# FlyCole/Dream2Real

Hardware: AMD Instinct MI355X
Metric: candidate renders scored/sec (640x360) (higher is better)
Workload: dtype bf16 + fp16 NeRF MLP operands (fp32 accumulate; the library's default: the reference's tiny-cuda-nn operand type, same MFMA rate; --opt mlp_f16=0 = bf16 operands)

## Files before the change

dream2real_amd/_lib.py:

```python
from __future__ import annotations

import ctypes as C
import os

import numpy as np

_HERE = os.path.dirname(os.path.abspath(__file__))
LIB_PATH = os.path.join(_HERE, "libd2r.so")
ABI_VERSION = 10

_int, _u32, _i64, _u64, _size, _f32, _f64, _str, _ptr = (C.c_int, C.c_uint32, C.c_int64, C.c_uint64, C.c_size_t, C.c_float, C.c_double,
                                                          C.c_char_p, C.c_void_p)
PROTOTYPES = {
    "d2r_abi_version": (_int, ()),
    "d2r_ctx_create": (_int, (_int, _ptr)),
    "d2r_ctx_destroy": (None, (_ptr,)),
    "d2r_ctx_set_stream": (_int, (_ptr, _ptr)),
    "d2r_ctx_synchronize": (_int, (_ptr,)),
    "d2r_last_error": (_str, (_ptr,)),
    "d2r_nerf_create": (_int, (_ptr, _ptr, _ptr)),
    "d2r_nerf_destroy": (None, (_ptr,)),
    "d2r_nerf_load_ingp": (_int, (_ptr, _ptr, _size, _ptr, _ptr, _ptr, _u32)),
    "d2r_ingp_inspect": (_int, (_ptr, _size, _ptr, _size, _ptr)),
    "d2r_ingp_validate": (_int, (_ptr, _size, _ptr)),
# ... 69 lines not shown
    "d2r_png_read_grey": (_int, (_str, _u32, _u32, _u32, _ptr)),
    "d2r_scene_bound_masks": (_int, (_ptr, _ptr, _u32, _u32, _u32, _ptr, _ptr, _ptr, _u32, _ptr, _ptr)),
    "d2r_masks_prune": (_int, (_ptr, _int, _ptr, _ptr, _ptr, _u32, _u32, _u32, _ptr, _ptr, _ptr, _u32, _ptr)),
    "d2r_masks_components": (_int, (_ptr, _ptr, _ptr, _u32, _u32, _ptr, _ptr, _ptr)),
    "d2r_masks_lut": (_int, (_ptr, _ptr, _ptr, _u32, _u32, _u32, _ptr, _ptr, _ptr)),
    "d2r_masks_census": (_int, (_ptr, _ptr, _u32, _u32, _u32, _ptr)),
    "d2r_masks_get_timing": (_int, (_ptr, _ptr)),
    "d2r_thumbs_plan": (_int, (_ptr, _ptr, _ptr, _ptr, _u32, _u32, _u32, _u32, _ptr, _ptr, _ptr, _ptr)),
    "d2r_thumbs_fill": (_int, (_ptr, _ptr, _ptr, _u64)),
    "d2r_thumbs_blur_bits": (_int, (_ptr, _ptr, _u32, _u32, _u32, _ptr)),
    "d2r_thumbs_get_timing": (_int, (_ptr, _ptr)),
    "d2r_proposals_labels": (_int, (_ptr, _ptr, _ptr, _u32, _u32, _u32, _ptr, _ptr, _ptr)),
    "d2r_proposals_get_timing": (_int, (_ptr, _ptr)),
    "d2r_labeltrack_grid": (_int, (_ptr, _ptr, _ptr, _ptr)),
    "d2r_labeltrack_scan": (_int, (_ptr, _ptr, _ptr, _u32, _u32, _u32, _ptr, _ptr, _ptr, _ptr, _ptr, _ptr, _ptr, _ptr, _ptr)),
    "d2r_labeltrack_get_timing": (_int, (_ptr, _ptr)),
    "d2r_geoprop_masks": (_int, (_ptr, _ptr, _ptr, _ptr, _u32, _u32, _ptr, _ptr, _ptr, _ptr, _ptr, _ptr, _ptr)),
    "d2r_geoprop_get_timing": (_int, (_ptr, _ptr)),
}
EXPORTS = list(PROTOTYPES)


class D2RError(RuntimeError):
    pass


class NerfDesc(C.Structure):
    _fields_ = [("n_levels", C.c_uint32), ("n_features", C.c_uint32), ("level_scale", C.c_void_p),
                ("level_res", C.c_void_p), ("level_size", C.c_void_p), ("level_offset", C.c_void_p),
                ("n_entries", C.c_uint32), ("grid_fp16", C.c_void_p), ("dw1_fp16", C.c_void_p),
                ("dw2_fp16", C.c_void_p), ("cw1_fp16", C.c_void_p), ("cw2_fp16", C.c_void_p),
                ("cw3_fp16", C.c_void_p), ("occupancy_bits", C.c_void_p), ("aabb_scale", C.c_uint32),
                ("render_aabb", C.c_float * 6)]


class ViewC(C.Structure):
    _fields_ = [("width", C.c_uint32), ("height", C.c_uint32), ("focal", C.c_float * 2),
                ("center", C.c_float * 2), ("scale", C.c_float), ("offset", C.c_float * 3),
                ("background", C.c_float * 4), ("min_transmittance", C.c_float),
                ("near_distance", C.c_float), ("lens_mode", C.c_uint32), ("lens_params", C.c_float * 4)]


class ClipDesc(C.Structure):
    _fields_ = [("image_size", C.c_uint32), ("patch_size", C.c_uint32), ("hidden_size", C.c_uint32),
                ("num_layers", C.c_uint32), ("num_heads", C.c_uint32), ("mlp_size", C.c_uint32),
                ("proj_dim", C.c_uint32)]


class TextDesc(C.Structure):
    _fields_ = [("vocab_size", C.c_uint32), ("context_length", C.c_uint32), ("hidden_size", C.c_uint32),
                ("num_layers", C.c_uint32), ("num_heads", C.c_uint32), ("mlp_size", C.c_uint32),
                ("proj_dim", C.c_uint32)]


class PhysParams(C.Structure):
    _fields_ = [("sample_res", C.c_uint32 * 6), ("init_pose", C.c_float * 16), ("table_z", C.c_float),
                ("unsup_thresh", C.c_float), ("gravity", C.c_float * 3), ("perturb", C.c_float),
                ("stability_check", C.c_int32), ("disallow_regrasp", C.c_int32), ("margin", C.c_float)]


class IngpView(C.Structure):
    _fields_ = [("fx", C.c_double), ("fy", C.c_double), ("cx", C.c_double), ("cy", C.c_double), ("w", C.c_uint32), ("h", C.c_uint32),
                ("lens_mode", C.c_uint32), ("lens_params", C.c_float * 4)]


class IngpInfo(C.Structure):
    _fields_ = [("n_levels", C.c_uint32), ("n_features", C.c_uint32), ("aabb_scale", C.c_uint32),
                ("has_background", C.c_int32), ("dataset_scale", C.c_double), ("dataset_offset", C.c_double * 3),
                ("background_color", C.c_float * 4), ("n_views", C.c_uint32), ("n_views_written", C.c_uint32),
                ("n_unknown_keys", C.c_uint32), ("render_with_lens_distortion", C.c_int32)]


class PcdView(C.Structure):
    _fields_ = [("width", C.c_uint32), ("height", C.c_uint32), ("fx", C.c_float), ("fy", C.c_float), ("cx", C.c_float),
                ("cy", C.c_float), ("point_size", C.c_float), ("near", C.c_float)]


class FrameSink(C.Structure):
    _fields_ = [("png_dir", C.c_char_p), ("png_first_index", C.c_uint32), ("png_threads", C.c_int32), ("png_level", C.c_int32)]


class RenderStats(C.Structure):
    _fields_ = [("rays_total", C.c_uint64), ("rays_alive", C.c_uint64), ("samples", C.c_uint64),
                ("wave_iters", C.c_uint64), ("l0_tokens", C.c_uint64), ("l0_touched", C.c_uint64)]


class Timing(C.Structure):
    _fields_ = [("march_ms", C.c_double), ("march_launches", C.c_uint64), ("raygen_ms", C.c_double),
                ("raygen_launches", C.c_uint64), ("prep_ms", C.c_double), ("prep_launches", C.c_uint64),
                ("clip_ms", C.c_double), ("clip_launches", C.c_uint64), ("sort_ms", C.c_double), ("sort_launches", C.c_uint64),
                ("vit_qkv_ms", C.c_double), ("vit_qkv_launches", C.c_uint64), ("vit_attn_ms", C.c_double), ("vit_attn_launches", C.c_uint64),
                ("vit_out_ms", C.c_double), ("vit_out_launches", C.c_uint64), ("vit_fc1_ms", C.c_double), ("vit_fc1_launches", C.c_uint64),
                ("vit_fc2_ms", C.c_double), ("vit_fc2_launches", C.c_uint64)]


COMM_ID_BYTES = 128

_lib = None


def load() -> C.CDLL:
    global _lib
    if _lib is not None:
        return _lib
    if not os.path.exists(LIB_PATH):
        raise D2RError(f"{LIB_PATH} is missing: build it with __graft_entry__.build() "
                       "(make -C dream2real_amd/csrc); there is no CPU fallback")
    try:
        import torch
    except ImportError:
        pass
    lib = C.CDLL(LIB_PATH)
    for name, (restype, argtypes) in PROTOTYPES.items():
        fn = getattr(lib, name)
        fn.restype, fn.argtypes = restype, argtypes
    if lib.d2r_abi_version() != ABI_VERSION:
        raise D2RError("libd2r.so ABI version mismatch")
    _lib = lib
    return lib


def ingp_inspect(data: bytes) -> str:
    lib = load()
    need = C.c_size_t(0)
    check(lib.d2r_ingp_inspect(data, len(data), None, 0, C.byref(need)))
    buf = C.create_string_buffer(need.value)
    check(lib.d2r_ingp_inspect(data, len(data), buf, need.value, None))
    return buf.value.decode("utf-8", "replace")


def png_write(rgb, path: str, level: int = -1):
    a = np.ascontiguousarray(rgb, np.uint8)
    assert a.ndim == 3 and a.shape[2] == 3
    check(load().d2r_png_write(ptr(a), a.shape[1], a.shape[0], os.fsencode(path), level))


def png_write_batch(frames, out_dir: str, first_index: int = 0, threads: int = 0, level: int = -1):
    a = np.ascontiguousarray(frames, np.uint8)
    assert a.ndim == 4 and a.shape[3] == 3
    check(load().d2r_png_write_batch(ptr(a), a.shape[0], a.shape[2], a.shape[1], os.fsencode(out_dir), first_index, threads, level))


def png_write_batch_bg(frames, background, out_dir: str, first_index: int = 0, threads: int = 0):
    a = np.ascontiguousarray(frames, np.uint8)
    b = np.ascontiguousarray(background, np.uint8)
    assert a.ndim == 4 and a.shape[3] == 3 and b.shape == a.shape[1:]
    check(load().d2r_png_write_batch_bg(ptr(a), a.shape[0], a.shape[2], a.shape[1], ptr(b), os.fsencode(out_dir), first_index, threads))


def png_write_channels(pixels, path: str, level: int = -1):
    a = np.ascontiguousarray(pixels, np.uint8)
    if a.ndim == 2:
        a = a[:, :, None]
    if a.ndim != 3 or a.shape[2] not in (1, 3, 4):
        raise ValueError(f"expected [h,w], [h,w,3] or [h,w,4], got shape {a.shape}")
    check(load().d2r_png_write_channels(ptr(a), a.shape[1], a.shape[0], a.shape[2], os.fsencode(path), level))


def png_info(path: str):
    v = [C.c_uint32(0) for _ in range(4)]
    check(load().d2r_png_info(os.fsencode(path), *[C.byref(x) for x in v]))
    return tuple(int(x.value) for x in v)


def png_read_rgb(path: str, size=None) -> np.ndarray:
    w, h = size or png_info(path)[:2]
    out = np.empty((h, w, 3), np.uint8)
# ... 286 lines not shown
```

dream2real_amd/csrc/api.hip:

```cpp
#include <math.h>
#include <string.h>

#include <algorithm>
#include <chrono>

#include "d2r_internal.h"
#include "pngio.h"

struct d2r_clip;
int d2r_launch_preprocess(d2r_ctx *, d2r_clip *, const uint8_t *frames_dev, uint32_t n, uint32_t w, uint32_t h,
                          int rot90, uint16_t *patches_dev, float *pixel_values_dev, const void *rects_dev = nullptr,
                          const uint16_t *bg_patches_dev = nullptr, bool touched_only = false);
bool d2r_clip_l0_supported(const d2r_ctx *, const d2r_clip *);
int d2r_clip_forward(d2r_ctx *, const d2r_clip *, const uint16_t *patches_dev, uint32_t n, const float *text_dev,
                     uint32_t C, float logit_scale, float *logits_dev, float *embeds_dev, const ClipL0Reuse *reuse = nullptr);
int d2r_clip_layer0_background(d2r_ctx *, const d2r_clip *, const uint16_t *bg_patches_dev, ClipL0Reuse *out);
int d2r_launch_patchify(d2r_ctx *, const d2r_clip *, const float *pv_dev, uint32_t n, uint16_t *patches_dev);
size_t d2r_clip_patch_bytes(const d2r_clip *, uint32_t n);
int d2r_launch_eval_points(d2r_ctx *, const d2r_nerf *, const float *xyz, const float *dirs, uint32_t n, float *out);
uint32_t d2r_clip_image_size(const d2r_clip *);
uint32_t d2r_clip_proj_dim(const d2r_clip *);
uint32_t d2r_clip_max_images(const d2r_clip *);
uint32_t d2r_clip_tokens(const d2r_clip *);

uint32_t d2r_pass_size(const d2r_ctx *ctx, const d2r_clip *clip, size_t px)
{
    uint64_t per = (uint64_t)std::max<int64_t>(1, ctx->chunk);
    if (clip) per = std::min<uint64_t>(per, d2r_clip_max_images(clip));
    if (px) per = std::min<uint64_t>(per, std::max<uint64_t>(1, 0xffffffffull / px));
    return (uint32_t)per;
}

static thread_local std::string g_err;

int d2r_fail(d2r_ctx *ctx, int code, const std::string &msg)
{
    if (ctx) ctx->err = msg;
    g_err = msg;
    return code;
}

hipStream_t d2r_stream(const d2r_ctx *ctx) { return ctx->stream; }

int d2r_reserve(d2r_ctx *ctx, d2r_ctx::Buf &b, size_t bytes)
{
    if (bytes <= b.cap) return D2R_OK;
    if (b.p) {
        D2R_HIP(ctx, hipStreamSynchronize(ctx->stream));
        (void)hipFree(b.p);
        b.p = nullptr;
        b.cap = 0;
    }
    size_t want = bytes + bytes / 8 + 256;
    if (hipMalloc(&b.p, want) != hipSuccess) {
        b.p = nullptr;
        return d2r_fail(ctx, D2R_ERR_MEMORY, "hipMalloc(" + std::to_string(want) + ") failed");
    }
    b.cap = want - 64;
    D2R_HIP(ctx, hipMemsetAsync(b.p, 0, want, ctx->stream));
    return D2R_OK;
}

uint32_t d2r_frame_pass_size(uint32_t per, size_t px)
{
    const uint64_t fit = std::max<uint64_t>(64, (1ull << 30) / (px * 3));
    uint64_t p = std::min<uint64_t>(per, fit);
    if (p >= 256) p -= p % 256;
    return (uint32_t)std::max<uint64_t>(1, p);
}

int d2r_upload_text(d2r_ctx *ctx, const d2r_clip *clip, const float *text, uint32_t C)
{
    if (!text || C == 0 || C > 1024) return d2r_fail(ctx, D2R_ERR_INVALID, "bad text embeddings");
    size_t bytes = (size_t)C * d2r_clip_proj_dim(clip) * 4;
    int rc = d2r_reserve(ctx, ctx->text, bytes);
    if (rc) return rc;
    const uint32_t slot = ctx->text_turn++ & 1u;
    if (ctx->text_ev[slot]) D2R_HIP(ctx, hipEventSynchronize(ctx->text_ev[slot]));
    else D2R_HIP(ctx, hipEventCreateWithFlags(&ctx->text_ev[slot], hipEventDisableTiming));
    if (ctx->text_host_cap[slot] < bytes) {
        if (ctx->text_host[slot]) (void)hipHostFree(ctx->text_host[slot]);
        ctx->text_host[slot] = nullptr;
        ctx->text_host_cap[slot] = 0;
        if (hipHostMalloc(&ctx->text_host[slot], bytes + 4096, hipHostMallocDefault) != hipSuccess)
            return d2r_fail(ctx, D2R_ERR_MEMORY, "hipHostMalloc failed for the text staging buffer");
        ctx->text_host_cap[slot] = bytes + 4096;
    }
    memcpy(ctx->text_host[slot], text, bytes);
    D2R_HIP(ctx, hipMemcpyAsync(ctx->text.p, ctx->text_host[slot], bytes, hipMemcpyHostToDevice, ctx->stream));
    D2R_HIP(ctx, hipEventRecord(ctx->text_ev[slot], ctx->stream));
    return D2R_OK;
}

int d2r_score_frames_chunked(d2r_ctx *ctx, const d2r_clip *clip, uint32_t n, uint32_t w, uint32_t h, int rot90, uint32_t C,
                             float logit_scale, const std::function<int(uint32_t, uint32_t)> &fill, float *logits_out,
                             float *embeds_out, uint8_t *frames_out)
{
    if (n == 0) return D2R_OK;
    const size_t fb = (size_t)w * h * 3;
    const uint32_t D = d2r_clip_proj_dim(clip);
    const uint32_t per = d2r_pass_size(ctx, clip, 0), cap = std::min(per, n);
    int rc;
    if ((rc = d2r_reserve(ctx, ctx->frames, (size_t)cap * fb))) return rc;
    if ((rc = d2r_reserve(ctx, ctx->clipws[6], d2r_clip_patch_bytes(clip, cap)))) return rc;
    if ((rc = d2r_reserve(ctx, ctx->logits, (size_t)cap * (C + D) * 4))) return rc;
    for (uint32_t c0 = 0; c0 < n; c0 += per) {
        const uint32_t nc = std::min(per, n - c0);
        float *lg = (float *)ctx->logits.p, *em = lg + (size_t)nc * C;
        if ((rc = fill(c0, nc))) return rc;
        if ((rc = d2r_launch_preprocess(ctx, (d2r_clip *)clip, (const uint8_t *)ctx->frames.p, nc, w, h, rot90,
                                        (uint16_t *)ctx->clipws[6].p, nullptr)))
            return rc;
        if ((rc = d2r_clip_forward(ctx, clip, (const uint16_t *)ctx->clipws[6].p, nc, (const float *)ctx->text.p, C,
                                   logit_scale, lg, em)))
            return rc;
        D2R_HIP(ctx, hipMemcpyAsync(logits_out + (size_t)c0 * C, lg, (size_t)nc * C * 4, hipMemcpyDeviceToHost, ctx->stream));
        if (embeds_out)
            D2R_HIP(ctx, hipMemcpyAsync(embeds_out + (size_t)c0 * D, em, (size_t)nc * D * 4, hipMemcpyDeviceToHost, ctx->stream));
        if (frames_out)
            D2R_HIP(ctx, hipMemcpyAsync(frames_out + (size_t)c0 * fb, ctx->frames.p, (size_t)nc * fb, hipMemcpyDeviceToHost, ctx->stream));
        D2R_HIP(ctx, hipStreamSynchronize(ctx->stream));
    }
    return D2R_OK;
}

struct Option {
    const char *key;
    int64_t d2r_ctx::*member;
    enum Kind { FLAG, RANGE, FREE } kind;
    int64_t lo, hi;
    unsigned flags;
    int (*hook)(d2r_ctx *, int64_t value);
};
enum { OPT_READ_ONLY = 1 };

static int opt_march_threads(d2r_ctx *ctx, int64_t value)
{
    if (value % 64)
        return d2r_fail(ctx, D2R_ERR_INVALID, "march_threads must be 0 (auto) or a multiple of 64 up to " + std::to_string(D2R_MARCH_THREADS) + " (the size the marcher was compiled for)");
    return D2R_OK;
}

static int opt_timing(d2r_ctx *ctx, int64_t)
{
    ctx->ev_used = 0;
    ctx->ev_pairs.clear();
    return D2R_OK;
}

static const Option g_options[] = {
    {"chunk", &d2r_ctx::chunk, Option::RANGE, 1, 16384},
    {"march_compact", &d2r_ctx::march_compact, Option::RANGE, 0, 1},
    {"refill_min", &d2r_ctx::refill_min, Option::RANGE, 1, 64},
    {"ln_fold", &d2r_ctx::ln_fold, Option::RANGE, 0, 4},
    {"gemm_nsplit", &d2r_ctx::gemm_nsplit, Option::FREE},
    {"prep_reuse", &d2r_ctx::prep_reuse, Option::FLAG},
    {"cls_last", &d2r_ctx::cls_last, Option::FLAG},
    {"vit_fp8", &d2r_ctx::vit_fp8, Option::FLAG},
    {"l0_reuse", &d2r_ctx::l0_reuse, Option::FLAG},
    {"attn_rem", &d2r_ctx::attn_rem, Option::RANGE, 0, 4},
    {"overlap", &d2r_ctx::overlap, Option::FLAG},
    {"debug_fail_chunk", &d2r_ctx::debug_fail_chunk, Option::FREE},
    {"ray_sort", &d2r_ctx::ray_sort, Option::RANGE, 0, 1},
    {"ray_sort_log2", &d2r_ctx::ray_sort_log2, Option::RANGE, 1, 4},
    {"march_threads", &d2r_ctx::march_threads, Option::RANGE, 0, D2R_MARCH_THREADS, 0, opt_march_threads},
    {"march_threads_auto_mib", &d2r_ctx::march_threads_auto_mib, Option::RANGE, 0, 1 << 20},
    {"march_blocks", &d2r_ctx::march_blocks, Option::RANGE, 0, 65535},
    {"gbrick_slots", &d2r_ctx::gbrick_slots, Option::RANGE, 0, 8},
    {"brick_slots_total", &d2r_ctx::brick_slots_total, Option::RANGE, 0, 8},
    {"lds_slots_max", &d2r_ctx::lds_slots_max, Option::RANGE, 0, 5},
    {"gbrick_max_mib", &d2r_ctx::gbrick_max_mib, Option::RANGE, 0, 512},
    {"mlp_f16", &d2r_ctx::mlp_f16, Option::FLAG},
    {"render_arith", &d2r_ctx::render_arith, Option::RANGE, 0, 2},
    {"bricks", &d2r_ctx::use_bricks, Option::FLAG},
    {"raygen_rect", &d2r_ctx::raygen_rect, Option::FLAG},
    {"timing", &d2r_ctx::timing, Option::RANGE, 0, 2, 0, opt_timing},
    {"march_lds_slots", &d2r_ctx::last_march_nb, Option::FREE, 0, 0, OPT_READ_ONLY},
    {"march_hbm_brick_slots", &d2r_ctx::last_march_ngb, Option::FREE, 0, 0, OPT_READ_ONLY},
    {"march_hbm_brick_bytes", &d2r_ctx::last_march_gbrick_bytes, Option::FREE, 0, 0, OPT_READ_ONLY},
    {"march_threads_used", &d2r_ctx::last_march_threads, Option::FREE, 0, 0, OPT_READ_ONLY},
};

static const Option *find_option(const char *key)
{
    for (const Option &o : g_options)
        if (!strcmp(key, o.key)) return &o;
    return nullptr;
}

size_t d2r_ctx::timing_begin(int kind)
{
    if (!timing || (kind >= D2R_T_VIT_QKV && timing < 2)) return (size_t)-1;
    while (ev_pool.size() < ev_used + 2) {
        hipEvent_t e;
        if (hipEventCreate(&e) != hipSuccess) return (size_t)-1;
        ev_pool.push_back(e);
    }
    size_t b = ev_used, e = ev_used + 1;
    ev_used += 2;
    ev_pairs.push_back({kind, {b, e}});
    (void)hipEventRecord(ev_pool[b], stream);
    return ev_pairs.size() - 1;
}

void d2r_ctx::timing_end(size_t pair)
{
    if (pair == (size_t)-1) return;
    (void)hipEventRecord(ev_pool[ev_pairs[pair].second.second], stream);
}

extern "C" {

int d2r_abi_version(void) { return D2R_ABI_VERSION; }

int d2r_get_timing(d2r_ctx *ctx, d2r_timing *out)
{
    if (!ctx || !out) return d2r_fail(ctx, D2R_ERR_INVALID, "null argument");
    D2R_HIP(ctx, hipStreamSynchronize(ctx->stream));
    double ms[D2R_T_KINDS] = {};
    uint64_t n[D2R_T_KINDS] = {};
    for (auto &p : ctx->ev_pairs) {
        float t = 0.f;
        if (hipEventElapsedTime(&t, ctx->ev_pool[p.second.first], ctx->ev_pool[p.second.second]) == hipSuccess) {
            ms[p.first] += t;
            n[p.first]++;
        }
    }
    out->march_ms = ms[D2R_T_MARCH];   out->march_launches = n[D2R_T_MARCH];
    out->raygen_ms = ms[D2R_T_RAYGEN]; out->raygen_launches = n[D2R_T_RAYGEN];
    out->prep_ms = ms[D2R_T_PREP];     out->prep_launches = n[D2R_T_PREP];
    out->clip_ms = ms[D2R_T_CLIP];     out->clip_launches = n[D2R_T_CLIP];
    out->sort_ms = ms[D2R_T_SORT];     out->sort_launches = n[D2R_T_SORT];
    out->vit_qkv_ms = ms[D2R_T_VIT_QKV];   out->vit_qkv_launches = n[D2R_T_VIT_QKV];
    out->vit_attn_ms = ms[D2R_T_VIT_ATTN]; out->vit_attn_launches = n[D2R_T_VIT_ATTN];
    out->vit_out_ms = ms[D2R_T_VIT_OUT];   out->vit_out_launches = n[D2R_T_VIT_OUT];
    out->vit_fc1_ms = ms[D2R_T_VIT_FC1];   out->vit_fc1_launches = n[D2R_T_VIT_FC1];
    out->vit_fc2_ms = ms[D2R_T_VIT_FC2];   out->vit_fc2_launches = n[D2R_T_VIT_FC2];
    ctx->ev_used = 0;
    ctx->ev_pairs.clear();
    return D2R_OK;
}

const char *d2r_last_error(d2r_ctx *ctx) { return ctx ? ctx->err.c_str() : g_err.c_str(); }

int d2r_ctx_create(int device, d2r_ctx **out)
{
    if (!out) return d2r_fail(nullptr, D2R_ERR_INVALID, "null out pointer");
    int n = 0;
    if (hipGetDeviceCount(&n) != hipSuccess || n <= 0)
        return d2r_fail(nullptr, D2R_ERR_DEVICE, "no HIP device: libd2r has no CPU path");
    if (device < 0 || device >= n) return d2r_fail(nullptr, D2R_ERR_INVALID, "device index out of range");
    hipDeviceProp_t prop;
    if (hipGetDeviceProperties(&prop, device) != hipSuccess)
        return d2r_fail(nullptr, D2R_ERR_DEVICE, "hipGetDeviceProperties failed");
    if (strncmp(prop.gcnArchName, "gfx950", 6) != 0)
        return d2r_fail(nullptr, D2R_ERR_DEVICE, std::string("libd2r is built for gfx950 only, found ") + prop.gcnArchName);
    if (hipSetDevice(device) != hipSuccess) return d2r_fail(nullptr, D2R_ERR_DEVICE, "hipSetDevice failed");
    d2r_ctx *c = new d2r_ctx();
    c->device = device;
    c->n_cu = prop.multiProcessorCount > 0 ? prop.multiProcessorCount : 256;
    int xcc = 0;
    if (hipDeviceGetAttribute(&xcc, hipDeviceAttributeNumberOfXccs, device) == hipSuccess && xcc > 0 && c->n_cu % xcc == 0)
        c->n_xcd = xcc;
    else
        c->n_xcd = c->n_cu % 8 == 0 ? 8 : 1;
    if (hipStreamCreateWithFlags(&c->own_stream, hipStreamNonBlocking) != hipSuccess) {
        delete c;
        return d2r_fail(nullptr, D2R_ERR_DEVICE, "hipStreamCreate failed");
    }
    c->stream = c->own_stream;
    *out = c;
    return D2R_OK;
}

void d2r_ctx_destroy(d2r_ctx *c)
{
    if (!c) return;
    hipSetDevice(c->device);
    hipStreamSynchronize(c->stream);
    (void)d2r_comm_destroy(c);
    if (c->render_stream) hipStreamSynchronize(c->render_stream);
    if (c->copy_stream) hipStreamSynchronize(c->copy_stream);
    delete c->pool;
    d2r_ctx::Buf *bufs[] = {&c->cams, &c->queue, &c->queue2, &c->sort_counts, &c->counters, &c->frames, &c->rgba, &c->depth, &c->poses,
                            &c->text, &c->logits, &c->pix, &c->bg_rgba, &c->bg_depth, &c->bg_u8, &c->rects, &c->bg_patches, &c->rect_ws, &c->lens_tab,
                            &c->patches2, &c->frames2, &c->bg_l0, &c->l0_a1, &c->l0_q2, &c->l0_misc,
                            &c->pcd_mats, &c->pcd_bg_keys, &c->pcd_bg_frame, &c->pcd_cols,
                            &c->tv_mats, &c->tv_bg_frame, &c->tv_bg_depth, &c->tv_depth, &c->ct_in, &c->ct_ws, &c->lt_in, &c->lt_ws, &c->gp_in, &c->gp_ws,
                            &c->mv_in, &c->mv_recs, &c->mv_queue, &c->mv_shade, &c->mv_keys, &c->mv_out,
                            &c->mask_in, &c->mask_out, &c->mask_ws, &c->thumb_in, &c->thumb_ws, &c->thumb_out,
                            &c->prop_in, &c->prop_ws, &c->prop_out};
    for (auto *b : bufs)
        if (b->p) hipFree(b->p);
    for (auto &b : c->clipws)
        if (b.p) hipFree(b.p);
    for (hipEvent_t e : c->ev_pool) (void)hipEventDestroy(e);
    for (int k = 0; k < 2; k++) {
        if (c->text_ev[k]) (void)hipEventDestroy(c->text_ev[k]);
        if (c->text_host[k]) (void)hipHostFree(c->text_host[k]);
    }
    hipEvent_t evs[] = {c->ev_fork, c->ev_prep[0], c->ev_prep[1], c->ev_clip[0], c->ev_clip[1], c->ev_march[0], c->ev_march[1],
                        c->ev_copy[0], c->ev_copy[1]};
    for (hipEvent_t e : evs)
        if (e) (void)hipEventDestroy(e);
    for (int k = 0; k < 2; k++)
        if (c->frame_host[k]) (void)hipHostFree(c->frame_host[k]);
    if (c->render_stream) (void)hipStreamDestroy(c->render_stream);
    if (c->copy_stream) (void)hipStreamDestroy(c->copy_stream);
    (void)hipStreamDestroy(c->own_stream);
    delete c;
}

int d2r_ctx_set_stream(d2r_ctx *ctx, void *s)
{
    if (!ctx) return d2r_fail(nullptr, D2R_ERR_INVALID, "null ctx");
    hipStreamSynchronize(ctx->stream);
    ctx->stream = s ? (hipStream_t)s : ctx->own_stream;
    return D2R_OK;
}

int d2r_ctx_synchronize(d2r_ctx *ctx)
{
    if (!ctx) return d2r_fail(nullptr, D2R_ERR_INVALID, "null ctx");
    D2R_HIP(ctx, hipStreamSynchronize(ctx->stream));
    return D2R_OK;
}

int d2r_ctx_set_option(d2r_ctx *ctx, const char *key, int64_t value)
{
    if (!ctx || !key) return d2r_fail(ctx, D2R_ERR_INVALID, "null argument");
    const Option *o = find_option(key);
    if (!o) return d2r_fail(ctx, D2R_ERR_INVALID, std::string("unknown option ") + key);
    if (o->flags & OPT_READ_ONLY) return d2r_fail(ctx, D2R_ERR_INVALID, std::string("option ") + key + " is a read-back and cannot be set");
    if (o->kind == Option::RANGE && (value < o->lo || value > o->hi))
        return d2r_fail(ctx, D2R_ERR_INVALID, std::string(key) + " must be in [" + std::to_string(o->lo) + ", " + std::to_string(o->hi) + "]");
    int rc;
    if (o->hook && (rc = o->hook(ctx, value))) return rc;
    ctx->*(o->member) = o->kind == Option::FLAG ? (int64_t)(value != 0) : value;
    return D2R_OK;
}

int d2r_ctx_get_option(d2r_ctx *ctx, const char *key, int64_t *value)
{
    if (!ctx || !key || !value) return d2r_fail(ctx, D2R_ERR_INVALID, "null argument");
    const Option *o = find_option(key);
    if (!o) return d2r_fail(ctx, D2R_ERR_INVALID, std::string("unknown option ") + key);
    *value = ctx->*(o->member);
    return D2R_OK;
}

int d2r_get_render_stats(d2r_ctx *ctx, d2r_render_stats *out)
{
    if (!ctx || !out) return d2r_fail(ctx, D2R_ERR_INVALID, "null argument");
    *out = ctx->stats;
    return D2R_OK;
}


static float half_to_float(uint16_t h)
{
    uint32_t sign = (uint32_t)(h & 0x8000u) << 16, exp = (h >> 10) & 0x1fu, man = h & 0x3ffu, bits;
    if (exp == 0) {
        if (man == 0) bits = sign;
        else {
            int e = -1;
            do { man <<= 1; e++; } while (!(man & 0x400u));
            bits = sign | ((uint32_t)(127 - 15 - e) << 23) | ((man & 0x3ffu) << 13);
        }
    } else if (exp == 31) bits = sign | 0x7f800000u | (man << 13);
    else bits = sign | ((exp + 127 - 15) << 23) | (man << 13);
    float f;
    memcpy(&f, &bits, 4);
    return f;
}

static uint16_t float_to_bf16(float f)
{
    uint32_t b;
    memcpy(&b, &f, 4);
    if ((b & 0x7fffffffu) > 0x7f800000u) return (uint16_t)((b >> 16) | 0x40);
    b += 0x7fffu + ((b >> 16) & 1u);
    return (uint16_t)(b >> 16);
}

static void build_frag(std::vector<uint16_t> &dst, bool f16, int frag, const uint16_t *w, int n_out, int n_in, int mtile,
                       int s, int kind, int col_base = 0)
{
    for (int lane = 0; lane < 64; lane++) {
        int i = lane & 31, hi = lane >> 5, row = mtile * 32 + i;
// ... 376 lines not shown
            return rc;
        if ((rc = d2r_launch_render(ctx, fg, V, (const float *)ctx->cams.p, nc, true, nullptr, nullptr, (uint8_t *)ctx->frames.p)))
            return rc;
        D2R_HIP(ctx, hipMemcpyAsync(frames_out + (size_t)c0 * px * 3, ctx->frames.p, (size_t)nc * px * 3, hipMemcpyDeviceToHost, ctx->stream));
        if ((rc = fetch_stats(ctx, (uint64_t)nc * px, true))) return rc;
    }
    return D2R_OK;
}


int d2r_clip_score_frames(d2r_ctx *ctx, const d2r_clip *clip, const uint8_t *frames, uint32_t n, uint32_t w,
                          uint32_t h, int rot90, const float *text_embeds, uint32_t C, float logit_scale,
                          float *logits_out, float *embeds_out)
{
    if (!ctx || !clip || !frames || !logits_out) return d2r_fail(ctx, D2R_ERR_INVALID, "null argument");
    D2R_HIP(ctx, hipSetDevice(ctx->device));
    int rc = d2r_upload_text(ctx, clip, text_embeds, C);
    if (rc) return rc;
    const size_t fb = (size_t)w * h * 3;
    auto fill = [&](uint32_t c0, uint32_t nc) {
        D2R_HIP(ctx, hipMemcpyAsync(ctx->frames.p, frames + (size_t)c0 * fb, (size_t)nc * fb, hipMemcpyHostToDevice, ctx->stream));
        return (int)D2R_OK;
    };
    return d2r_score_frames_chunked(ctx, clip, n, w, h, rot90, C, logit_scale, fill, logits_out, embeds_out, nullptr);
}

int d2r_clip_preprocess(d2r_ctx *ctx, const d2r_clip *clip, const uint8_t *frames, uint32_t n, uint32_t w,
                        uint32_t h, int rot90, float *pixel_values_out)
{
    if (!ctx || !clip || !frames || !pixel_values_out) return d2r_fail(ctx, D2R_ERR_INVALID, "null argument");
    D2R_HIP(ctx, hipSetDevice(ctx->device));
    const size_t px = (size_t)w * h, S = d2r_clip_image_size(clip);
    int rc;
    if ((rc = d2r_reserve(ctx, ctx->frames, (size_t)n * px * 3))) return rc;
    if ((rc = d2r_reserve(ctx, ctx->pix, (size_t)n * 3 * S * S * 4))) return rc;
    D2R_HIP(ctx, hipMemcpyAsync(ctx->frames.p, frames, (size_t)n * px * 3, hipMemcpyHostToDevice, ctx->stream));
    if ((rc = d2r_launch_preprocess(ctx, (d2r_clip *)clip, (const uint8_t *)ctx->frames.p, n, w, h, rot90, nullptr,
                                    (float *)ctx->pix.p)))
        return rc;
    D2R_HIP(ctx, hipMemcpyAsync(pixel_values_out, ctx->pix.p, (size_t)n * 3 * S * S * 4, hipMemcpyDeviceToHost, ctx->stream));
    D2R_HIP(ctx, hipStreamSynchronize(ctx->stream));
    return D2R_OK;
}

int d2r_clip_embed_pixels(d2r_ctx *ctx, const d2r_clip *clip, const float *pixel_values, uint32_t n,
                          float *embeds_out)
{
    if (!ctx || !clip || !pixel_values || !embeds_out) return d2r_fail(ctx, D2R_ERR_INVALID, "null argument");
    D2R_HIP(ctx, hipSetDevice(ctx->device));
    const size_t S = d2r_clip_image_size(clip);
    const uint32_t D = d2r_clip_proj_dim(clip);
    int rc;
    const uint32_t per = d2r_pass_size(ctx, clip, 0);
    for (uint32_t c0 = 0; c0 < n; c0 += per) {
        uint32_t nc = std::min(per, n - c0);
        if ((rc = d2r_reserve(ctx, ctx->pix, (size_t)nc * 3 * S * S * 4))) return rc;
        if ((rc = d2r_reserve(ctx, ctx->clipws[6], d2r_clip_patch_bytes(clip, nc)))) return rc;
        if ((rc = d2r_reserve(ctx, ctx->logits, (size_t)nc * D * 4))) return rc;
        if ((rc = d2r_reserve(ctx, ctx->text, (size_t)D * 4))) return rc;
        D2R_HIP(ctx, hipMemcpyAsync(ctx->pix.p, pixel_values + (size_t)c0 * 3 * S * S, (size_t)nc * 3 * S * S * 4, hipMemcpyHostToDevice, ctx->stream));
        if ((rc = d2r_launch_patchify(ctx, clip, (const float *)ctx->pix.p, nc, (uint16_t *)ctx->clipws[6].p))) return rc;
        if ((rc = d2r_clip_forward(ctx, clip, (const uint16_t *)ctx->clipws[6].p, nc, (const float *)ctx->text.p, 0, 1.0f,
                                   nullptr, (float *)ctx->logits.p)))
            return rc;
        D2R_HIP(ctx, hipMemcpyAsync(embeds_out + (size_t)c0 * D, ctx->logits.p, (size_t)nc * D * 4, hipMemcpyDeviceToHost, ctx->stream));
        D2R_HIP(ctx, hipStreamSynchronize(ctx->stream));
    }
    return D2R_OK;
}


struct StreamSwap {
    d2r_ctx *c;
    hipStream_t saved;
    StreamSwap(d2r_ctx *ctx, hipStream_t s) : c(ctx), saved(ctx->stream) { ctx->stream = s; }
    ~StreamSwap() { c->stream = saved; }
};

static int ensure_pipeline(d2r_ctx *ctx, bool need_copy)
{
    if (!ctx->render_stream) D2R_HIP(ctx, hipStreamCreateWithFlags(&ctx->render_stream, hipStreamNonBlocking));
    if (need_copy && !ctx->copy_stream) D2R_HIP(ctx, hipStreamCreateWithFlags(&ctx->copy_stream, hipStreamNonBlocking));
    hipEvent_t *all[] = {&ctx->ev_fork, &ctx->ev_prep[0], &ctx->ev_prep[1], &ctx->ev_clip[0], &ctx->ev_clip[1],
                         &ctx->ev_march[0], &ctx->ev_march[1], &ctx->ev_copy[0], &ctx->ev_copy[1]};
    for (hipEvent_t *e : all)
        if (!*e) D2R_HIP(ctx, hipEventCreateWithFlags(e, hipEventDisableTiming));
    return D2R_OK;
}

static void dispatch_frames(d2r_ctx *ctx, int b, uint32_t c0, uint32_t nc, uint32_t W, uint32_t H, uint8_t *frames_out,
                            const d2r_frame_sink *sink)
{
    const uint8_t *src = (const uint8_t *)ctx->frame_host[b];
    const size_t fb = (size_t)W * H * 3;
    if (sink && sink->png_dir) {
        const std::string dir(sink->png_dir);
        const uint32_t first = sink->png_first_index + c0;
        const int level = sink->png_level;
        const std::shared_ptr<const D2rPngBase> base = level < 0 ? ctx->png_base : nullptr;
        for (uint32_t i = 0; i < nc; i++) {
            if (base) ctx->pool->submit(b, [=](std::string &err) { return d2r_png_write_file_delta(*base, src + fb * i, d2r_png_name(dir, first + i), err); });
            else ctx->pool->submit(b, [=](std::string &err) { return d2r_png_write_file(src + fb * i, W, H, level, d2r_png_name(dir, first + i), err); });
        }
    }
    if (frames_out) {
        const uint32_t step = std::max<uint32_t>(1, (uint32_t)((32u << 20) / fb));
        for (uint32_t i = 0; i < nc; i += step) {
            const uint32_t m = std::min(step, nc - i);
            uint8_t *dst = frames_out + ((size_t)c0 + i) * fb;
            ctx->pool->submit(b, [=](std::string &) { memcpy(dst, src + fb * i, fb * m); return 0; });
        }
    }
}

static int render_score_body(d2r_ctx *ctx, const d2r_nerf *fg, const d2r_clip *clip, const d2r_view *view,
                             const float *obj_pose_now, const float *cam_pose, const float *poses_dev, uint32_t K,
                             uint32_t C, float logit_scale, float *logits_dev, uint8_t *frames_out, const d2r_frame_sink *sink)
{
    int rc;
    ViewParams V = d2r_view_params(view);
    const size_t px = (size_t)V.W * V.H;
    const bool to_host = frames_out || (sink && sink->png_dir);
    uint32_t per = d2r_pass_size(ctx, clip, px);
    if (to_host) per = d2r_frame_pass_size(per, px);
    const uint32_t nchunks = (K + per - 1) / per;
    ctx->last_pass = per;
    ctx->last_chunks = nchunks;
    const uint32_t cap = std::min(per, K);
    const bool two = ctx->overlap != 0 && nchunks > 1;
    if ((rc = ensure_pipeline(ctx, to_host))) return rc;
    const size_t patch_bytes = d2r_clip_patch_bytes(clip, cap);
    if ((rc = d2r_reserve(ctx, ctx->cams, (size_t)cap * 48))) return rc;
    if ((rc = d2r_reserve_render(ctx, (size_t)cap * px))) return rc;
    if ((rc = d2r_lens_table(ctx, V))) return rc;
    if ((rc = d2r_reserve(ctx, ctx->frames, (size_t)cap * px * 3))) return rc;
    if ((rc = d2r_reserve(ctx, ctx->clipws[6], patch_bytes))) return rc;
    if (two && (rc = d2r_reserve(ctx, ctx->patches2, patch_bytes))) return rc;
    if (to_host && nchunks > 1 && (rc = d2r_reserve(ctx, ctx->frames2, (size_t)cap * px * 3))) return rc;
    if ((rc = d2r_reserve(ctx, ctx->counters, 64 + 32 * (size_t)nchunks))) return rc;
    if (to_host) {
        const size_t hb = (size_t)cap * px * 3;
        for (int b = 0; b < (nchunks > 1 ? 2 : 1); b++)
            if (ctx->frame_host_cap[b] < hb) {
                if (ctx->frame_host[b]) (void)hipHostFree(ctx->frame_host[b]);
                ctx->frame_host[b] = nullptr;
                ctx->frame_host_cap[b] = 0;
                if (hipHostMalloc(&ctx->frame_host[b], hb, hipHostMallocDefault) != hipSuccess)
                    return d2r_fail(ctx, D2R_ERR_MEMORY, "hipHostMalloc(" + std::to_string(hb) + ") failed for the frame staging buffer");
                ctx->frame_host_cap[b] = hb;
            }
        if (sink && sink->png_dir && sink->png_level < 0 && !ctx->png_base && ctx->bg_u8.p && ctx->bg_w == V.W && ctx->bg_h == V.H) {
            std::vector<uint8_t> bg(px * 3);
            D2R_HIP(ctx, hipMemcpy(bg.data(), ctx->bg_u8.p, px * 3, hipMemcpyDeviceToHost));
            ctx->png_base = d2r_png_base_build(bg.data(), V.W, V.H);
        }
        const int want = sink && sink->png_threads > 0 ? sink->png_threads : d2r_default_io_threads();
        if (!ctx->pool || ctx->pool->size() != want) {
            delete ctx->pool;
            ctx->pool = new D2rJobPool(want);
        }
    }
    const bool reuse_bg = ctx->prep_reuse && ctx->raygen_rect && ctx->bg_w == V.W && ctx->bg_h == V.H && ctx->bg_u8.p;
    if (reuse_bg) {
        if ((rc = d2r_reserve(ctx, ctx->rects, (size_t)cap * 16 * 2))) return rc;
        if (ctx->bg_patches_for != (const void *)clip) {
            if ((rc = d2r_reserve(ctx, ctx->bg_patches, d2r_clip_patch_bytes(clip, 1)))) return rc;
            if ((rc = d2r_launch_preprocess(ctx, (d2r_clip *)clip, (const uint8_t *)ctx->bg_u8.p, 1, V.W, V.H, 1,
                                            (uint16_t *)ctx->bg_patches.p, nullptr)))
                return rc;
            ctx->bg_patches_for = (const void *)clip;
            ctx->bg_l0_for = nullptr;
        }
    }
    ClipL0Reuse l0{};
    const bool use_l0 = reuse_bg && ctx->l0_reuse && d2r_clip_l0_supported(ctx, clip);
    if (use_l0) {
        if (ctx->bg_l0_for != (const void *)clip) {
            rc = d2r_clip_layer0_background(ctx, clip, (const uint16_t *)ctx->bg_patches.p, &ctx->bg_l0_desc);
            if (rc == D2R_OK) ctx->bg_l0_for = (const void *)clip;
            else if (rc != D2R_ERR_UNSUPPORTED) return rc;
        }
        if (ctx->bg_l0_for == (const void *)clip) {
            l0 = ctx->bg_l0_desc;
            l0.w = V.W;
            l0.h = V.H;
            l0.rects = ctx->rects.p;
        }
    }
    ctx->stats = d2r_render_stats{};
    hipStream_t main = ctx->stream, rs = two ? ctx->render_stream : main, xs = ctx->copy_stream;
    if (rs != main) {
        D2R_HIP(ctx, hipEventRecord(ctx->ev_fork, main));
        D2R_HIP(ctx, hipStreamWaitEvent(rs, ctx->ev_fork, 0));
    }
    uint32_t prev_c0 = 0, prev_nc = 0;
    int prev_b = -1;
    for (uint32_t c0 = 0, ci = 0; c0 < K; c0 += per, ci++) {
        const uint32_t nc = std::min(per, K - c0);
        const int b = (int)(ci & 1u), pb = two ? b : 0, fbuf = (to_host && nchunks > 1) ? b : 0;
        uint8_t *frames_dev = (uint8_t *)(fbuf ? ctx->frames2.p : ctx->frames.p);
        uint16_t *patches = (uint16_t *)(pb ? ctx->patches2.p : ctx->clipws[6].p);
        void *rects = reuse_bg ? (void *)((uint8_t *)ctx->rects.p + (size_t)pb * cap * 16) : nullptr;
        if (to_host && ci >= 2) ctx->pool->wait(b);
        {
            StreamSwap sw(ctx, rs);
            if (to_host && ci >= 2) D2R_HIP(ctx, hipStreamWaitEvent(rs, ctx->ev_copy[b], 0));
            if (two && ci >= 2) D2R_HIP(ctx, hipStreamWaitEvent(rs, ctx->ev_clip[pb], 0));
            if ((rc = d2r_launch_cameras_virtual(ctx, V, obj_pose_now, cam_pose, poses_dev + (size_t)c0 * 16, nc, (float *)ctx->cams.p)))
                return rc;
            if ((rc = d2r_launch_render(ctx, fg, V, (const float *)ctx->cams.p, nc, true, nullptr, nullptr, frames_dev, rects)))
                return rc;
            D2R_HIP(ctx, hipMemcpyAsync((uint8_t *)ctx->counters.p + 64 + 32 * (size_t)ci, ctx->counters.p, 32,
                                        hipMemcpyDeviceToDevice, rs));
            if (ctx->debug_fail_chunk >= 0 && (int64_t)ci == ctx->debug_fail_chunk) {
                ctx->debug_fail_chunk = -1;
                return d2r_fail(ctx, D2R_ERR_DEVICE, "injected fault in chunk " + std::to_string(ci) + " (option debug_fail_chunk)");
            }
            size_t tp = ctx->timing_begin(D2R_T_PREP);
            if ((rc = d2r_launch_preprocess(ctx, (d2r_clip *)clip, frames_dev, nc, V.W, V.H, 1, patches, nullptr, rects,
                                            reuse_bg ? (const uint16_t *)ctx->bg_patches.p : nullptr, l0.rects != nullptr)))
                return rc;
            ctx->timing_end(tp);
            if (to_host) {
                D2R_HIP(ctx, hipEventRecord(ctx->ev_march[b], rs));
                D2R_HIP(ctx, hipStreamWaitEvent(xs, ctx->ev_march[b], 0));
                D2R_HIP(ctx, hipMemcpyAsync(ctx->frame_host[b], frames_dev, (size_t)nc * px * 3, hipMemcpyDeviceToHost, xs));
                D2R_HIP(ctx, hipEventRecord(ctx->ev_copy[b], xs));
            }
            if (two) D2R_HIP(ctx, hipEventRecord(ctx->ev_prep[pb], rs));
        }
        if (two) D2R_HIP(ctx, hipStreamWaitEvent(main, ctx->ev_prep[pb], 0));
        size_t tc = ctx->timing_begin(D2R_T_CLIP);
        if (l0.rects) {
            l0.rects = rects;
            l0.touched_out = (uint32_t *)((uint8_t *)ctx->counters.p + 64 + 32 * (size_t)ci) + 6;
        }
        if ((rc = d2r_clip_forward(ctx, clip, patches, nc, (const float *)ctx->text.p, C, logit_scale,
                                   logits_dev + (size_t)c0 * C, nullptr, l0.rects ? &l0 : nullptr)))
            return rc;
        ctx->timing_end(tc);
        if (two) D2R_HIP(ctx, hipEventRecord(ctx->ev_clip[pb], main));
        if (to_host) {
            if (prev_b >= 0) {
                D2R_HIP(ctx, hipEventSynchronize(ctx->ev_copy[prev_b]));
                dispatch_frames(ctx, prev_b, prev_c0, prev_nc, V.W, V.H, frames_out, sink);
            }
            prev_b = b;
            prev_c0 = c0;
            prev_nc = nc;
        }
    }
    if (to_host) {
        const bool io_debug = getenv("D2R_IO_DEBUG") != nullptr;
        const auto t0 = std::chrono::steady_clock::now();
        auto ms = [&]() { return std::chrono::duration<double, std::milli>(std::chrono::steady_clock::now() - t0).count(); };
        if (prev_b >= 0) {
            D2R_HIP(ctx, hipEventSynchronize(ctx->ev_copy[prev_b]));
            if (io_debug) fprintf(stderr, "[d2r io] last chunk's frames on the host after %.1f ms\n", ms());
            dispatch_frames(ctx, prev_b, prev_c0, prev_nc, V.W, V.H, frames_out, sink);
        }
        if (io_debug) {
            D2R_HIP(ctx, hipStreamSynchronize(main));
            fprintf(stderr, "[d2r io] device work done after %.1f ms\n", ms());
        }
        ctx->pool->wait(-1);
        if (io_debug) fprintf(stderr, "[d2r io] %u frames in %u chunks: files written %.1f ms after the last launch (%d threads)\n", K, nchunks, ms(), ctx->pool->size());
        std::string err;
        int prc = ctx->pool->take_error(err);
        D2R_HIP(ctx, hipStreamSynchronize(main));
        if (prc) return d2r_fail(ctx, prc, err);
    }
    ctx->stats.rays_total = (uint64_t)K * px;
    ctx->stats.l0_tokens = l0.rects ? (uint64_t)K * (d2r_clip_tokens(clip) - 1) : 0;
    return D2R_OK;
}

static int render_score_core(d2r_ctx *ctx, const d2r_nerf *fg, const d2r_clip *clip, const d2r_view *view,
                             const float *obj_pose_now, const float *cam_pose, const float *poses_dev, uint32_t K,
                             uint32_t C, float logit_scale, float *logits_dev, uint8_t *frames_out, const d2r_frame_sink *sink)
{
    const int rc = render_score_body(ctx, fg, clip, view, obj_pose_now, cam_pose, poses_dev, K, C, logit_scale, logits_dev, frames_out, sink);
    if (rc == D2R_OK) return rc;
    const std::string first = ctx->err;
    if (ctx->render_stream) (void)hipStreamSynchronize(ctx->render_stream);
    if (ctx->copy_stream) (void)hipStreamSynchronize(ctx->copy_stream);
    (void)hipStreamSynchronize(ctx->stream);
    if (ctx->pool) {
        ctx->pool->wait(-1);
        std::string dropped;
        (void)ctx->pool->take_error(dropped);
    }
    (void)hipGetLastError();
    ctx->last_chunks = 0;
    ctx->err = first;
    return rc;
}

static int check_render_score_args(d2r_ctx *ctx, const d2r_nerf *fg, const d2r_clip *clip, const d2r_view *view,
                                   const float *obj_pose_now, const float *cam_pose, const void *poses, const void *logits,
                                   const d2r_frame_sink *sink)
{
    if (!ctx || !fg || !clip || !obj_pose_now || !cam_pose || !poses || !logits)
        return d2r_fail(ctx, D2R_ERR_INVALID, "null argument");
    if (sink && sink->png_dir && (sink->png_level > 9 || sink->png_threads > 1024))
        return d2r_fail(ctx, D2R_ERR_INVALID, "bad d2r_frame_sink (png_level 0..9 or negative for the default, png_threads <= 1024)");
    return check_view(ctx, view);
}

int d2r_render_score(d2r_ctx *ctx, const d2r_nerf *fg, const d2r_clip *clip, const d2r_view *view,
                     const float *obj_pose_now, const float *cam_pose, const float *obj_poses_dev, uint32_t K,
                     const float *text_embeds, uint32_t C, float logit_scale, float *logits_dev, uint8_t *frames_out)
{
    int rc = check_render_score_args(ctx, fg, clip, view, obj_pose_now, cam_pose, obj_poses_dev, logits_dev, nullptr);
    if (rc) return rc;
    D2R_HIP(ctx, hipSetDevice(ctx->device));
    if ((rc = d2r_upload_text(ctx, clip, text_embeds, C))) return rc;
    return render_score_core(ctx, fg, clip, view, obj_pose_now, cam_pose, obj_poses_dev, K, C, logit_scale, logits_dev,
                             frames_out, nullptr);
}

int d2r_render_score_host(d2r_ctx *ctx, const d2r_nerf *fg, const d2r_clip *clip, const d2r_view *view,
                          const float *obj_pose_now, const float *cam_pose, const float *obj_poses, uint32_t K,
// ... 47 lines not shown
```

dream2real_amd/csrc/clip.hip:

```cpp
#include "d2r_internal.h"

#include <type_traits>

#include <math.h>
#include <stdio.h>
#include <stdlib.h>

#include <algorithm>
#include <deque>
#include <mutex>

typedef __bf16 bf16x8 __attribute__((ext_vector_type(8)));
typedef float f32x16 __attribute__((ext_vector_type(16)));
typedef float f32x4 __attribute__((ext_vector_type(4)));

struct ClipWeights {
    const uint16_t *w_patch;
    const float *cls, *pos;
    const float *pre_w, *pre_b;
    struct Layer {
        const float *ln1_w, *ln1_b, *ln2_w, *ln2_b;
        const uint16_t *w_qkv, *w_o, *w_fc1, *w_fc2;
        const float *b_qkv, *b_o, *b_fc1, *b_fc2;
        const uint16_t *wf_qkv = nullptr, *wf_fc1 = nullptr;
        const float *cs_qkv = nullptr, *cs_fc1 = nullptr;
        const float *bf_qkv = nullptr, *bf_fc1 = nullptr;
    };
    const float *post_w, *post_b;
    const float *proj;
};

struct ResampleTables {
    const int *bounds_h;
    const int *kk_h;
    const int *bounds_v;
    const int *kk_v;
    int ks_h, ks_v;
    int need_h, need_v;
    int iw, ih;
    int rw, rh;
    int left, top;
    int max_rows;
};

struct PrepCache {
    uint32_t w, h;
    int rot90;
    ResampleTables R;
};

struct d2r_clip {
    d2r_ctx *ctx;
    d2r_clip_desc desc;
    uint32_t T, Kp, Kp_pad;
    std::vector<void *> allocs;
    ClipWeights w;
    std::vector<ClipWeights::Layer> layers;
    std::deque<PrepCache> prep;
    std::mutex prep_mu;
    struct F8Layer { const uint8_t *w_qkv, *w_o, *w_fc1, *w_fc2; float s_qkv, s_o, s_fc1, s_fc2; };
    std::vector<F8Layer> f8;
    std::mutex f8_mu;
};

__device__ __forceinline__ uint16_t f2bf(float x)
{
    union { __bf16 b; uint16_t u; } c;
    c.b = (__bf16)x;
    return c.u;
}
__device__ __forceinline__ uint32_t pack2(float a, float b)
{
    typedef __bf16 bf16x2 __attribute__((ext_vector_type(2)));
    union { bf16x2 v; uint32_t u; } r;
    r.v[0] = (__bf16)a;
    r.v[1] = (__bf16)b;
    return r.u;
}
__device__ __forceinline__ float wave_sum(float v)
{
#pragma unroll
    for (int o = 32; o > 0; o >>= 1) v += __shfl_xor(v, o);
    return v;
}


#define PRECISION_BITS 22
__device__ __forceinline__ uint32_t clip8(int v)
{
    v >>= PRECISION_BITS;
    return (uint32_t)min(max(v, 0), 255);
}

__global__ __launch_bounds__(256) void k_preprocess(const uint8_t *__restrict__ frames, uint32_t w, uint32_t h,
                                                    int rot90, ResampleTables R, uint32_t S, uint32_t P,
                                                    uint32_t band, uint16_t *__restrict__ patches,
                                                    uint32_t Kp_pad, float *__restrict__ pixel_values,
                                                    const int4 *__restrict__ rects, const uint16_t *__restrict__ bg_patches, int touched_only)
{
    extern __shared__ __attribute__((aligned(16))) uint8_t tmp[];
    const uint32_t img = blockIdx.y;
    const uint32_t row0 = blockIdx.x * band;
    const uint32_t nrows = min(band, S - row0);
    uint32_t x_lo = 0, x_n = S;
    if (rects && bg_patches && patches && !pixel_values && band == P) {
        int ys, ye;
        if (R.need_v) {
            ys = R.bounds_v[2 * (R.top + row0)];
            const int lastrow = R.top + row0 + nrows - 1;
            ye = R.bounds_v[2 * lastrow] + R.bounds_v[2 * lastrow + 1];
        } else {
            ys = R.top + row0;
            ye = ys + nrows;
        }
        const int4 rc = rects[img];
        const int rlo = rot90 ? (int)w - 1 - rc.z : rc.y, rhi = rot90 ? (int)w - 1 - rc.x : rc.w;
        const bool untouched = rc.x > rc.z || rc.y > rc.w || rhi < ys || rlo >= ye;
        if (touched_only) {
            if (untouched) return;
            const int clo = rot90 ? rc.y : rc.x, chi = rot90 ? rc.w : rc.z;
            uint32_t p_lo = S / P, p_hi = 0;
            for (uint32_t pcol = 0; pcol < S / P; pcol++) {
                int xs, xe;
                if (R.need_h) {
                    xs = R.bounds_h[2 * (R.left + pcol * P)];
                    const int last = R.left + pcol * P + P - 1;
                    xe = R.bounds_h[2 * last] + R.bounds_h[2 * last + 1];
                } else { xs = R.left + pcol * P; xe = xs + P; }
                if (!(chi < xs || clo >= xe)) { p_lo = min(p_lo, pcol); p_hi = max(p_hi, pcol + 1); }
            }
            if (p_lo >= p_hi) return;
// ... 1257 lines not shown
    }
    const float mu = s * inv_d, r = 1.0f / sqrtf(fmaxf(q * inv_d - mu * mu, 0.f) + 1e-5f);
    AB[row] = make_float2(r, -r * mu);
}


__global__ __launch_bounds__(256) void k_ln_q8(const uint16_t *__restrict__ Xhi, const float2 *__restrict__ AB, const float *__restrict__ gamma,
                                               const float *__restrict__ beta, uint32_t M_pad, uint32_t d, uint8_t *__restrict__ A8,
                                               uint8_t *__restrict__ SA)
{
    const uint32_t planes = d >> 6, items = planes * (M_pad >> 6);
    const uint32_t c8 = (threadIdx.x & 7) * 8, r = threadIdx.x >> 3;
    for (uint32_t it = blockIdx.x; it < items; it += gridDim.x) {
        const uint32_t p = it % planes, b = it / planes;
        const float4 g0 = *(const float4 *)(gamma + p * 64 + c8), g1 = *(const float4 *)(gamma + p * 64 + c8 + 4);
        const float4 e0 = *(const float4 *)(beta + p * 64 + c8), e1 = *(const float4 *)(beta + p * 64 + c8 + 4);
        const float gm[8] = {g0.x, g0.y, g0.z, g0.w, g1.x, g1.y, g1.z, g1.w}, bt[8] = {e0.x, e0.y, e0.z, e0.w, e1.x, e1.y, e1.z, e1.w};
        uint4 h[2];
        float2 ab[2];
#pragma unroll
        for (int ii = 0; ii < 2; ii++) {
            const size_t row = (size_t)b * 64 + r + 32 * ii;
            h[ii] = *(const uint4 *)(Xhi + ((size_t)p * M_pad + row) * 64 + c8);
            ab[ii] = AB[row];
        }
#pragma unroll
        for (int ii = 0; ii < 2; ii++) {
            const size_t row = (size_t)b * 64 + r + 32 * ii;
            const uint32_t hw[4] = {h[ii].x, h[ii].y, h[ii].z, h[ii].w};
            float f[8];
            float am = 0.f;
#pragma unroll
            for (int e = 0; e < 8; e++) {
                const float x = (e & 1) ? bf_hi(hw[e >> 1]) : bf_lo(hw[e >> 1]);
                f[e] = fmaf(fmaf(x, ab[ii].x, ab[ii].y), gm[e], bt[e]);
                am = fmaxf(am, fabsf(f[e]));
            }
            const uint32_t sb = q8_scale_byte(row8_max(am));
            *(uint2 *)(A8 + (((size_t)p * M_pad + row) << 6) + c8) = q8_pack8(f, q8_inv_scale(sb));
            if ((threadIdx.x & 7) == 0) SA[q8_scale_off(M_pad, row, p)] = (uint8_t)sb;
        }
    }
}

__global__ __launch_bounds__(256) void k_amax_bf16(const uint16_t *__restrict__ W, size_t n, uint32_t *__restrict__ amax_bits)
{
    uint32_t m = 0;
    for (size_t i = (size_t)blockIdx.x * blockDim.x + threadIdx.x; i < n; i += (size_t)gridDim.x * blockDim.x) m = max(m, (uint32_t)(W[i] & 0x7fffu) << 16);
    for (int o = 32; o > 0; o >>= 1) m = max(m, (uint32_t)__shfl_xor((int)m, o));
    if ((threadIdx.x & 63) == 0) atomicMax(amax_bits, m);
}
__global__ __launch_bounds__(256) void k_quant_w8(const uint16_t *__restrict__ W, size_t n, const uint32_t *__restrict__ amax_bits,
                                                  uint8_t *__restrict__ W8)
{
    const float inv = q8_inv_scale(q8_scale_byte(__uint_as_float(*amax_bits)));
    for (size_t i = ((size_t)blockIdx.x * blockDim.x + threadIdx.x) * 4; i < n; i += (size_t)gridDim.x * blockDim.x * 4) {
        const uint2 w = *(const uint2 *)(W + i);
        uint32_t q = __builtin_amdgcn_cvt_pk_fp8_f32(bf_lo(w.x) * inv, bf_hi(w.x) * inv, 0, false);
        q = __builtin_amdgcn_cvt_pk_fp8_f32(bf_lo(w.y) * inv, bf_hi(w.y) * inv, q, true);
        *(uint32_t *)(W8 + i) = q;
    }
}
__global__ __launch_bounds__(256) void k_quant_rows_q8(const float *__restrict__ A, uint32_t M, uint32_t K, uint32_t M_pad, uint8_t *__restrict__ A8,
                                                       uint8_t *__restrict__ SA)
{
    const size_t t = (size_t)blockIdx.x * blockDim.x + threadIdx.x;
    const uint32_t per_row = K >> 3;
    const size_t row = t / per_row;
    if (row >= M_pad) return;
    const uint32_t col = (uint32_t)(t - row * per_row) * 8;
    float f[8];
    float am = 0.f;
#pragma unroll
    for (int e = 0; e < 8; e++) {
        f[e] = row < M ? A[row * K + col + e] : 0.f;
        am = fmaxf(am, fabsf(f[e]));
    }
    const uint32_t sb = q8_scale_byte(row8_max(am));
    *(uint2 *)(A8 + (((size_t)(col >> 6) * M_pad + row) << 6) + (col & 63)) = q8_pack8(f, q8_inv_scale(sb));
    if ((col & 63) == 0) SA[q8_scale_off(M_pad, row, col >> 6)] = (uint8_t)sb;
}


__global__ __launch_bounds__(256) void k_touch_list(const int4 *__restrict__ rects, uint32_t w, ResampleTables R, uint32_t S, uint32_t P,
                                                    uint32_t *__restrict__ cnt, uint32_t *__restrict__ list)
{
    __shared__ uint32_t ids[1024], n_ids, base;
    const uint32_t img = blockIdx.x, g = S / P, g2 = g * g;
    if (threadIdx.x == 0) n_ids = 0;
    __syncthreads();
    const int4 rc = rects[img];
    const bool empty = rc.x > rc.z || rc.y > rc.w;
    const int rlo = (int)w - 1 - rc.z, rhi = (int)w - 1 - rc.x, clo = rc.y, chi = rc.w;
    for (uint32_t p = threadIdx.x; p < g2 && !empty; p += blockDim.x) {
        const uint32_t pr = p / g, pcol = p - pr * g;
        int ys, ye, xs, xe;
        if (R.need_v) {
            ys = R.bounds_v[2 * (R.top + pr * P)];
            const int last = R.top + pr * P + P - 1;
            ye = R.bounds_v[2 * last] + R.bounds_v[2 * last + 1];
        } else { ys = R.top + pr * P; ye = ys + P; }
        if (R.need_h) {
            xs = R.bounds_h[2 * (R.left + pcol * P)];
            const int last = R.left + pcol * P + P - 1;
            xe = R.bounds_h[2 * last] + R.bounds_h[2 * last + 1];
        } else { xs = R.left + pcol * P; xe = xs + P; }
        if (!(rhi < ys || rlo >= ye || chi < xs || clo >= xe)) ids[atomicAdd(&n_ids, 1u)] = img * g2 + p;
    }
    __syncthreads();
    if (threadIdx.x == 0) base = n_ids ? atomicAdd(cnt, n_ids) : 0u;
    __syncthreads();
    for (uint32_t i = threadIdx.x; i < n_ids; i += blockDim.x) list[base + i] = ids[i];
}

__global__ __launch_bounds__(256) void k_gather_rows(const uint16_t *__restrict__ src, uint32_t row_elems, const uint32_t *__restrict__ list,
                                                     const uint32_t *__restrict__ cnt, uint16_t *__restrict__ out)
{
    const uint32_t lane = threadIdx.x & 63, n = *cnt, per = row_elems / 8;
    for (uint32_t i = blockIdx.x * 4 + (threadIdx.x >> 6); i < n; i += gridDim.x * 4) {
        const uint4 *s = (const uint4 *)(src + (size_t)list[i] * row_elems);
        uint4 *o = (uint4 *)(out + (size_t)i * row_elems);
        for (uint32_t c = lane; c < per; c += 64) o[c] = s[c];
    }
}

__global__ __launch_bounds__(256) void k_bcast_x0(const uint16_t *__restrict__ bg_hi, const uint8_t *__restrict__ bg_lo, const float2 *__restrict__ bg_ab,
                                                  uint32_t bg_rows, uint16_t *__restrict__ Xhi, uint8_t *__restrict__ Xlo, float2 *__restrict__ AB,
                                                  uint32_t rows, uint32_t M_pad, uint32_t T, uint32_t d)
{
    const uint32_t lane = threadIdx.x & 63, row = blockIdx.x * 4 + (threadIdx.x >> 6);
    if (row >= rows) return;
    const uint32_t t = row % T;
    for (uint32_t c8 = lane; c8 < d / 8; c8 += 64) {
        const uint32_t c = c8 * 8;
        *(uint4 *)(Xhi + ((size_t)(c >> 6) * M_pad + row) * 64 + (c & 63)) = *(const uint4 *)(bg_hi + ((size_t)(c >> 6) * bg_rows + t) * 64 + (c & 63));
        *(uint2 *)(Xlo + lo8_off(M_pad, row, c)) = *(const uint2 *)(bg_lo + lo8_off(bg_rows, t, c));
    }
    if (lane == 0) AB[row] = bg_ab[t];
}

__global__ __launch_bounds__(256) void k_bcast_qkv(const uint16_t *__restrict__ bg_qkv, uint32_t bg_rows, uint16_t *__restrict__ QKV, uint32_t rows,
                                                   uint32_t M_pad, uint32_t T, uint32_t planes)
{
    const size_t i = (size_t)blockIdx.x * blockDim.x + threadIdx.x;
    const size_t total = (size_t)planes * rows * 8;
    if (i >= total) return;
    const uint32_t piece = (uint32_t)(i & 7);
    const size_t pr = i >> 3;
    const uint32_t row = (uint32_t)(pr % rows), plane = (uint32_t)(pr / rows);
    *(uint4 *)(QKV + ((size_t)plane * M_pad + row) * 64 + piece * 8) = *(const uint4 *)(bg_qkv + ((size_t)plane * bg_rows + row % T) * 64 + piece * 8);
}

__global__ __launch_bounds__(256) void k_gather_operand_rows(const uint16_t *__restrict__ Xhi, const float2 *__restrict__ AB, uint32_t M_pad, uint32_t T,
                                                             const uint32_t *__restrict__ list, const uint32_t *__restrict__ cnt,
                                                             uint16_t *__restrict__ A2, float2 *__restrict__ AB2, uint32_t cap_pad, uint32_t d)
{
    const uint32_t lane = threadIdx.x & 63, n = *cnt;
    for (uint32_t i = blockIdx.x * 4 + (threadIdx.x >> 6); i < n; i += gridDim.x * 4) {
        const uint32_t e = list[i], bi = e / (T - 1), row = bi * T + 1 + (e - bi * (T - 1));
        for (uint32_t c8 = lane; c8 < d / 8; c8 += 64) {
            const uint32_t c = c8 * 8;
            *(uint4 *)(A2 + ((size_t)(c >> 6) * cap_pad + i) * 64 + (c & 63)) = *(const uint4 *)(Xhi + ((size_t)(c >> 6) * M_pad + row) * 64 + (c & 63));
        }
        if (lane == 0) AB2[i] = AB[row];
    }
}

__global__ __launch_bounds__(256) void k_scatter_qkv(const uint16_t *__restrict__ Q2, uint32_t cap_pad, const uint32_t *__restrict__ list,
                                                     const uint32_t *__restrict__ cnt, uint16_t *__restrict__ QKV, uint32_t M_pad, uint32_t T, uint32_t planes)
{
    const uint32_t lane = threadIdx.x & 63, n = *cnt;
    for (uint32_t i = blockIdx.x * 4 + (threadIdx.x >> 6); i < n; i += gridDim.x * 4) {
        const uint32_t e = list[i], bi = e / (T - 1), row = bi * T + 1 + (e - bi * (T - 1));
        for (uint32_t j = lane; j < planes * 8; j += 64) {
            const uint32_t plane = j >> 3, piece = j & 7;
            *(uint4 *)(QKV + ((size_t)plane * M_pad + row) * 64 + piece * 8) = *(const uint4 *)(Q2 + ((size_t)plane * cap_pad + i) * 64 + piece * 8);
        }
    }
}

__global__ void k_fold_ln_weight(const float *__restrict__ W, const float *__restrict__ gamma, const float *__restrict__ beta,
                                 const float *__restrict__ b, uint16_t *__restrict__ Wf, float *__restrict__ cs,
                                 float *__restrict__ bf, uint32_t N, uint32_t K, float scale = 1.0f)
{
    const uint32_t n = blockIdx.x * (blockDim.x >> 6) + (threadIdx.x >> 6), lane = threadIdx.x & 63;
    if (n >= N) return;
    float s = 0.f, t = 0.f;
    for (uint32_t k = lane; k < K; k += 64) {
        const float w = W[(size_t)n * K + k];
        const uint16_t h = f2bf(w * gamma[k] * scale);
        Wf[(size_t)n * K + k] = h;
        s += __uint_as_float((uint32_t)h << 16);
        t = fmaf(w, beta[k], t);
    }
    s = wave_sum(s);
// ... 765 lines not shown
    if (x < 1.0) return ((a + 2.0) * x - (a + 3.0)) * x * x + 1;
    if (x < 2.0) return (((x - 5) * x + 8) * x - 4) * a;
    return 0.0;
}

static int resample_coeffs(int in_size, int out_size, std::vector<int> &bounds, std::vector<int> &kk)
{
    double scale = (double)in_size / out_size, filterscale = scale < 1.0 ? 1.0 : scale;
    double support = 2.0 * filterscale;
    int ksize = (int)ceil(support) * 2 + 1;
    bounds.assign((size_t)out_size * 2, 0);
    kk.assign((size_t)out_size * ksize, 0);
    std::vector<double> k(ksize);
    for (int xx = 0; xx < out_size; xx++) {
        double center = (xx + 0.5) * scale, ww = 0.0, ss = 1.0 / filterscale;
        int xmin = (int)(center - support + 0.5);
        if (xmin < 0) xmin = 0;
        int xmax = (int)(center + support + 0.5);
        if (xmax > in_size) xmax = in_size;
        xmax -= xmin;
        for (int x = 0; x < xmax; x++) {
            k[x] = bicubic_filter((x + xmin - center + 0.5) * ss);
            ww += k[x];
        }
        for (int x = 0; x < ksize; x++) {
            double v = x < xmax ? (ww != 0.0 ? k[x] / ww : k[x]) : 0.0;
            kk[(size_t)xx * ksize + x] = v < 0 ? (int)(-0.5 + v * (1 << PRECISION_BITS))
                                               : (int)(0.5 + v * (1 << PRECISION_BITS));
        }
        bounds[xx * 2] = xmin;
        bounds[xx * 2 + 1] = xmax;
    }
    return ksize;
}

static int prep_tables(d2r_ctx *ctx, d2r_clip *clip, uint32_t w, uint32_t h, int rot90, const PrepCache **out)
{
    std::lock_guard<std::mutex> lock(clip->prep_mu);
    for (const PrepCache &pc : clip->prep)
        if (pc.w == w && pc.h == h && pc.rot90 == rot90) {
            *out = &pc;
            return D2R_OK;
        }
    const uint32_t S = clip->desc.image_size, P = clip->desc.patch_size;
    ResampleTables R{};
    R.iw = rot90 ? (int)h : (int)w;
    R.ih = rot90 ? (int)w : (int)h;
    int short_e = R.iw < R.ih ? R.iw : R.ih, long_e = R.iw < R.ih ? R.ih : R.iw;
    int new_long = (int)((double)S * long_e / short_e);
    R.rw = R.iw <= R.ih ? (int)S : new_long;
    R.rh = R.iw <= R.ih ? new_long : (int)S;
    R.need_h = R.rw != R.iw;
    R.need_v = R.rh != R.ih;
    R.left = (R.rw - (int)S) / 2;
    R.top = (R.rh - (int)S) / 2;
    std::vector<int> bh, kh, bv, kv;
    R.ks_h = resample_coeffs(R.iw, R.rw, bh, kh);
    R.ks_v = resample_coeffs(R.ih, R.rh, bv, kv);
    const uint32_t band = P;
    int max_rows = (int)band;
    if (R.need_v) {
        max_rows = 0;
        for (uint32_t r0 = 0; r0 < S; r0 += band) {
            uint32_t last = std::min(r0 + band, S) - 1;
            int y0 = bv[2 * (R.top + r0)], y1 = bv[2 * (R.top + last)] + bv[2 * (R.top + last) + 1];
            max_rows = std::max(max_rows, y1 - y0);
        }
    }
    R.max_rows = max_rows;
    std::vector<int> all;
    size_t o_bh = 0, o_kh = o_bh + bh.size(), o_bv = o_kh + kh.size(), o_kv = o_bv + bv.size();
    all.insert(all.end(), bh.begin(), bh.end());
    all.insert(all.end(), kh.begin(), kh.end());
    all.insert(all.end(), bv.begin(), bv.end());
    all.insert(all.end(), kv.begin(), kv.end());
    int *dev = nullptr;
    if (hipMalloc(&dev, all.size() * sizeof(int)) != hipSuccess) return d2r_fail(ctx, D2R_ERR_MEMORY, "hipMalloc failed");
    clip->allocs.push_back(dev);
    D2R_HIP(ctx, hipMemcpy(dev, all.data(), all.size() * sizeof(int), hipMemcpyHostToDevice));
    R.bounds_h = dev + o_bh;
    R.kk_h = dev + o_kh;
    R.bounds_v = dev + o_bv;
    R.kk_v = dev + o_kv;
    clip->prep.push_back(PrepCache{w, h, rot90, R});
    *out = &clip->prep.back();
    return D2R_OK;
}

int d2r_launch_preprocess(d2r_ctx *ctx, d2r_clip *clip, const uint8_t *frames_dev, uint32_t n, uint32_t w,
                          uint32_t h, int rot90, uint16_t *patches_dev, float *pixel_values_dev, const void *rects_dev,
                          const uint16_t *bg_patches_dev, bool touched_only)
{
    const uint32_t S = clip->desc.image_size, P = clip->desc.patch_size;
    const PrepCache *pc = nullptr;
    int rc = prep_tables(ctx, clip, w, h, rot90, &pc);
    if (rc) return rc;
    const ResampleTables &R = pc->R;
    const uint32_t band = P;
    size_t lds = (size_t)R.max_rows * S * 3;
    if (lds > 150 * 1024) return d2r_fail(ctx, D2R_ERR_UNSUPPORTED, "preprocess band does not fit in LDS");
    static PerDeviceOnce prep_attr;
    prep_attr.run(ctx->device, [] {
        (void)hipFuncSetAttribute((const void *)k_preprocess, hipFuncAttributeMaxDynamicSharedMemorySize, 150 * 1024);
    });
    hipLaunchKernelGGL(k_preprocess, dim3((S + band - 1) / band, n), dim3(256), lds, ctx->stream, frames_dev, w, h,
                       rot90, R, S, P, band, patches_dev, clip->Kp_pad, pixel_values_dev, (const int4 *)rects_dev, bg_patches_dev,
                       touched_only ? 1 : 0);
    D2R_HIP(ctx, hipGetLastError());
    return D2R_OK;
}

template <int EPI, int WGM, int WGN, int MT, int STAGES>
static int launch_gemm_cfg(d2r_ctx *ctx, const uint16_t *A, const uint16_t *W, const float *bias, void *C,
                           uint32_t M_real, uint32_t N, uint32_t K, const EpiAux &aux)
{
    constexpr uint32_t TBM = WGM * MT * 32, TBN = WGN * 64, LDS = STAGES * (TBM + TBN) * BK * 2;
    const uint32_t M_pad = round_up(M_real, BM);
    const uint32_t nwg = (M_pad / TBM) * (N / TBN);
    static PerDeviceOnce attr_set;
    attr_set.run(ctx->device, [] {
        (void)hipFuncSetAttribute((const void *)k_gemm<EPI, WGM, WGN, MT, STAGES>, hipFuncAttributeMaxDynamicSharedMemorySize, LDS);
    });
    hipLaunchKernelGGL((k_gemm<EPI, WGM, WGN, MT, STAGES>), dim3(aux.m_dev ? std::min<uint32_t>(nwg, (uint32_t)ctx->n_cu) : nwg), dim3(WGM * WGN * 64), LDS,
                       ctx->stream, A, W, bias, C, M_pad, N, K, (uint32_t)ctx->n_xcd, aux);
    D2R_HIP(ctx, hipGetLastError());
    return D2R_OK;
}

template <int EPI>
static int launch_gemm8(d2r_ctx *ctx, const uint16_t *A, const uint16_t *W, const float *bias, void *C, uint32_t M_real, uint32_t N, uint32_t K,
                        const EpiAux &aux)
{
    const uint32_t M_pad = round_up(M_real, BM);
    constexpr uint32_t LDS8 = 128 * 1024 + 8 * EP_WAVE_FLOATS * 4 + 8 * 1024;
    static PerDeviceOnce attr8;
    attr8.run(ctx->device, [] {
        if constexpr (EPI_IS_F8(EPI)) (void)hipFuncSetAttribute((const void *)k_gemm8f<EPI>, hipFuncAttributeMaxDynamicSharedMemorySize, LDS8);
        else (void)hipFuncSetAttribute((const void *)k_gemm8<EPI>, hipFuncAttributeMaxDynamicSharedMemorySize, LDS8);
    });
    const uint32_t nwg8 = (uint32_t)(ctx->n_cu / ctx->n_xcd * ctx->n_xcd);
    const uint32_t gn = N / 256;
    uint32_t ns = (uint32_t)ctx->gemm_nsplit;
    if (ns == 0) ns = 2;
    if (ns < 1 || (uint32_t)ctx->n_xcd % ns || (N / 256) % ns) ns = 1;
    if constexpr (EPI_IS_F8(EPI))
        hipLaunchKernelGGL((k_gemm8f<EPI>), dim3(nwg8), dim3(512), LDS8, ctx->stream, (const uint8_t *)A, (const uint8_t *)W, bias, C, M_pad, N, K,
                           (uint32_t)ctx->n_xcd, aux, (ns << 16) | gn);
    else
    hipLaunchKernelGGL((k_gemm8<EPI>), dim3(nwg8), dim3(512), LDS8, ctx->stream, A, W, bias, C, M_pad, N, K,
                       (uint32_t)ctx->n_xcd, aux, (ns << 16) | gn);
    D2R_HIP(ctx, hipGetLastError());
    return D2R_OK;
}

template <int EPI>
static int launch_gemm(d2r_ctx *ctx, const uint16_t *A, const uint16_t *W, const float *bias, void *C,
                       uint32_t M_real, uint32_t N, uint32_t K, const EpiAux &aux = EpiAux{})
{
    if (N % 128 || K % BK) return d2r_fail(ctx, D2R_ERR_UNSUPPORTED, "GEMM N must be a multiple of 128 and K of 64");
    if ((uint64_t)round_up(M_real, BM) * N >= (1ull << 32))
        return d2r_fail(ctx, D2R_ERR_UNSUPPORTED, "GEMM output too large for 32-bit indexing");
    if (EPI_IS_STATS(EPI) && (uint64_t)round_up(M_real, BM) * N * (EPI == EPI_RESID_STATS_F32X ? 4 : 2) >= (1ull << 32))
        return d2r_fail(ctx, D2R_ERR_UNSUPPORTED, "residual array too large for 32-bit byte offsets");
    if (EPI_IS_STATS(EPI) && aux.hm_rows != round_up(M_real, BM))
        return d2r_fail(ctx, D2R_ERR_INVALID, "residual + statistics epilogues write tile-major planes of M_pad rows");
    const uint64_t tiles256 = (uint64_t)(round_up(M_real, BM) / 256) * (N / 256);
    if (N % 256 == 0 && (N >= 2048 || tiles256 >= 1024)) {
// ... 107 lines not shown
    out->bg_hi = hi;
    out->bg_lo = lo;
    out->bg_ab = ab;
    out->bg_qkv = qkv;
    out->bg_rows = R;
    return D2R_OK;
}

static int ensure_f8_weights(d2r_ctx *ctx, d2r_clip *clip)
{
    std::lock_guard<std::mutex> lock(clip->f8_mu);
    if (!clip->f8.empty()) return D2R_OK;
    const d2r_clip_desc &D = clip->desc;
    const size_t d = D.hidden_size, mlp = D.mlp_size, nl = D.num_layers;
    const size_t sizes[4] = {3 * d * d, d * d, mlp * d, d * mlp};
    const size_t per_layer = sizes[0] + sizes[1] + sizes[2] + sizes[3];
    uint8_t *w8 = nullptr;
    uint32_t *amax = nullptr;
    if (hipMalloc(&w8, per_layer * nl) != hipSuccess || hipMalloc(&amax, nl * 4 * 4) != hipSuccess) {
        if (w8) (void)hipFree(w8);
        return d2r_fail(ctx, D2R_ERR_MEMORY, "hipMalloc failed for the fp8 weight copies");
    }
    clip->allocs.push_back(w8);
    clip->allocs.push_back(amax);
    D2R_HIP(ctx, hipMemsetAsync(amax, 0, nl * 16, ctx->stream));
    std::vector<d2r_clip::F8Layer> f8(nl);
    for (size_t l = 0; l < nl; l++) {
        const ClipWeights::Layer &L = clip->layers[l];
        const uint16_t *src[4] = {L.w_qkv, L.w_o, L.w_fc1, L.w_fc2};
        uint8_t *dst = w8 + l * per_layer;
        const uint8_t *out[4];
        for (int i = 0; i < 4; i++) {
            hipLaunchKernelGGL(k_amax_bf16, dim3(1024), dim3(256), 0, ctx->stream, src[i], sizes[i], amax + l * 4 + i);
            hipLaunchKernelGGL(k_quant_w8, dim3(1024), dim3(256), 0, ctx->stream, src[i], sizes[i], (const uint32_t *)(amax + l * 4 + i), dst);
            out[i] = dst;
            dst += sizes[i];
        }
        f8[l].w_qkv = out[0]; f8[l].w_o = out[1]; f8[l].w_fc1 = out[2]; f8[l].w_fc2 = out[3];
    }
    std::vector<uint32_t> bits(nl * 4);
    D2R_HIP(ctx, hipMemcpyAsync(bits.data(), amax, nl * 16, hipMemcpyDeviceToHost, ctx->stream));
    D2R_HIP(ctx, hipStreamSynchronize(ctx->stream));
    auto scale_of = [](uint32_t b) {
        const int e = (int)((b + 0x200000u) >> 23);
        const int byte = std::min(std::max(e - 8, 1), 253);
        return std::ldexp(1.0f, byte - 127);
    };
    for (size_t l = 0; l < nl; l++) {
        f8[l].s_qkv = scale_of(bits[l * 4 + 0]); f8[l].s_o = scale_of(bits[l * 4 + 1]);
        f8[l].s_fc1 = scale_of(bits[l * 4 + 2]); f8[l].s_fc2 = scale_of(bits[l * 4 + 3]);
    }
    clip->f8 = std::move(f8);
    return D2R_OK;
}

int d2r_clip_forward(d2r_ctx *ctx, const d2r_clip *clip, const uint16_t *patches_dev, uint32_t n,
                     const float *text_dev, uint32_t C, float logit_scale, float *logits_dev, float *embeds_dev,
                     const ClipL0Reuse *reuse)
{
    const d2r_clip_desc &D = clip->desc;
    const uint32_t d = D.hidden_size, T = clip->T, mlp = D.mlp_size;
    const uint32_t rows = n * T, rows_pad = round_up(rows, BM);
    const uint32_t prow = n * (T - 1);
    int rc;
    if ((rc = d2r_reserve(ctx, ctx->clipws[0], (size_t)round_up(prow, BM) * d * 4))) return rc;
    if ((rc = d2r_reserve(ctx, ctx->clipws[1], (size_t)rows_pad * d * 4))) return rc;
    if ((rc = d2r_reserve(ctx, ctx->clipws[2], (size_t)rows_pad * d * 2))) return rc;
    if ((rc = d2r_reserve(ctx, ctx->clipws[3], (size_t)rows_pad * 3 * d * 2))) return rc;
    if ((rc = d2r_reserve(ctx, ctx->clipws[4], (size_t)rows_pad * d * 2))) return rc;
    if ((rc = d2r_reserve(ctx, ctx->clipws[5], (size_t)rows_pad * mlp * 2))) return rc;
    float *patch_out = (float *)ctx->clipws[0].p, *X = (float *)ctx->clipws[1].p;
    uint16_t *Xn = (uint16_t *)ctx->clipws[2].p, *QKV = (uint16_t *)ctx->clipws[3].p;
    uint16_t *AO = (uint16_t *)ctx->clipws[4].p, *H = (uint16_t *)ctx->clipws[5].p;

    const int fold = (int)ctx->ln_fold;
    const bool l0 = reuse && reuse->rects;
    if (l0 && (!d2r_clip_l0_supported(ctx, clip) || T > reuse->bg_rows))
        return d2r_fail(ctx, D2R_ERR_INVALID, "d2r_clip_forward: layer-0 reuse requested for a model / option set that does not support it");
    uint32_t *l0_cnt = nullptr, *l0_list = nullptr;
    const uint32_t cap_pad = round_up(prow, BM);
    if (l0) {
        const PrepCache *pc = nullptr;
        if ((rc = prep_tables(ctx, (d2r_clip *)clip, reuse->w, reuse->h, 1, &pc))) return rc;
        if ((rc = d2r_reserve(ctx, ctx->l0_misc, 256 + (size_t)prow * 4 + (size_t)cap_pad * 8))) return rc;
        if ((rc = d2r_reserve(ctx, ctx->l0_a1, (size_t)cap_pad * clip->Kp_pad * 2))) return rc;
        if ((rc = d2r_reserve(ctx, ctx->l0_q2, (size_t)cap_pad * 3 * d * 2))) return rc;
        l0_cnt = (uint32_t *)ctx->l0_misc.p;
        l0_list = l0_cnt + 64;
        D2R_HIP(ctx, hipMemsetAsync(l0_cnt, 0, 4, ctx->stream));
        hipLaunchKernelGGL(k_touch_list, dim3(n), dim3(256), 0, ctx->stream, (const int4 *)reuse->rects, reuse->w, pc->R, D.image_size, D.patch_size, l0_cnt, l0_list);
        hipLaunchKernelGGL(k_gather_rows, dim3(2048), dim3(256), 0, ctx->stream, patches_dev, clip->Kp_pad, l0_list, l0_cnt, (uint16_t *)ctx->l0_a1.p);
        if (reuse->touched_out) D2R_HIP(ctx, hipMemcpyAsync(reuse->touched_out, l0_cnt, 4, hipMemcpyDeviceToDevice, ctx->stream));
        if (getenv("D2R_L0_DEBUG")) {
            uint32_t c = 0;
            (void)hipMemcpyAsync(&c, l0_cnt, 4, hipMemcpyDeviceToHost, ctx->stream);
            (void)hipStreamSynchronize(ctx->stream);
            fprintf(stderr, "[d2r l0_reuse] %u of %u patch tokens touched (%.1f %%)\n", c, prow, 100.0 * c / prow);
        }
        EpiAux a1{};
        a1.m_dev = l0_cnt;
        if ((rc = launch_gemm_cfg<EPI_F32, 4, 2, 2, 3>(ctx, (const uint16_t *)ctx->l0_a1.p, clip->w.w_patch, nullptr, patch_out, prow, d, clip->Kp_pad, a1))) return rc;
    } else if ((rc = launch_gemm<EPI_F32>(ctx, patches_dev, clip->w.w_patch, nullptr, patch_out, prow, d, clip->Kp_pad)))
        return rc;
    const bool cls_last = ctx->cls_last && D.num_layers >= 1 && T <= 1024 && round_up(n, BM) <= round_up(prow, BM);
    EpiAux out_tm{}, a_tm{};
    out_tm.hm_rows = rows_pad;
    a_tm.a_rs = 64;
    a_tm.a_ks = (uint32_t)64 * rows_pad;
    if ((uint64_t)64 * rows_pad >= (1ull << 32)) return d2r_fail(ctx, D2R_ERR_UNSUPPORTED, "activation plane too large for 32-bit indexing");
    if (fold == 0) {
        hipLaunchKernelGGL(k_embed_ln, dim3((rows + 3) / 4), dim3(256), 0, ctx->stream, patch_out, clip->w.cls,
                           clip->w.pos, clip->w.pre_w, clip->w.pre_b, X, rows, T, d, (uint16_t *)nullptr, (float2 *)nullptr, (uint16_t *)nullptr, rows_pad);
        for (uint32_t l = 0; l < D.num_layers; l++) {
            const ClipWeights::Layer &L = clip->layers[l];
            hipLaunchKernelGGL(k_layernorm, dim3((rows + 3) / 4), dim3(256), 0, ctx->stream, X, L.ln1_w, L.ln1_b, Xn,
                               rows, d);
            if ((rc = launch_gemm<EPI_BIAS_BF16>(ctx, Xn, L.w_qkv, L.b_qkv, QKV, rows, 3 * d, d, out_tm))) return rc;
            if (cls_last && l + 1 == D.num_layers) {
                if ((rc = last_block_cls(ctx, D, L, n, T, rows_pad, QKV, nullptr, X, nullptr, nullptr, patch_out, AO, Xn, H))) return rc;
                break;
            }
            launch_attention_vision(ctx, QKV, AO, T, d, rows_pad, D.num_heads, n);
            if ((rc = launch_gemm<EPI_BIAS_RESID_F32>(ctx, AO, L.w_o, L.b_o, X, rows, d, d, a_tm))) return rc;
            hipLaunchKernelGGL(k_layernorm, dim3((rows + 3) / 4), dim3(256), 0, ctx->stream, X, L.ln2_w, L.ln2_b, Xn,
                               rows, d);
            if ((rc = launch_gemm<EPI_BIAS_GELU_BF16>(ctx, Xn, L.w_fc1, L.b_fc1, H, rows, mlp, d, out_tm))) return rc;
            if ((rc = launch_gemm<EPI_BIAS_RESID_F32>(ctx, H, L.w_fc2, L.b_fc2, X, rows, d, mlp, a_tm))) return rc;
        }
        hipLaunchKernelGGL(k_head, dim3((n + HEAD_NI - 1) / HEAD_NI), dim3(HEAD_THREADS), 0, ctx->stream, cls_last ? patch_out : X, (const uint16_t *)nullptr, (const uint16_t *)nullptr, rows_pad,
                           (const uint32_t *)nullptr, cls_last ? 1u : T, d,
                           clip->w.post_w, clip->w.post_b, clip->w.proj, D.proj_dim, text_dev, C, logit_scale, logits_dev, embeds_dev, n);
        D2R_HIP(ctx, hipGetLastError());
        return D2R_OK;
    }
    const uint32_t np = d / 64;
    if ((rc = d2r_reserve(ctx, ctx->clipws[7], (size_t)rows_pad * np * 8 + (size_t)rows_pad * 8))) return rc;
    float2 *part = (float2 *)ctx->clipws[7].p, *AB = part + (size_t)rows_pad * np;
    const bool xf32 = fold == 3, split8 = fold == 4, split = fold == 1 || split8;
    const int lo8 = split8 ? 1 : 0;
    uint16_t *Xlo = split ? (uint16_t *)X : (uint16_t *)nullptr;
    if (l0) {
        hipLaunchKernelGGL(k_bcast_x0, dim3((rows + 3) / 4), dim3(256), 0, ctx->stream, reuse->bg_hi, reuse->bg_lo, reuse->bg_ab, reuse->bg_rows, Xn,
                           (uint8_t *)Xlo, AB, rows, rows_pad, T, d);
        hipLaunchKernelGGL(k_embed_ln, dim3(std::min<uint32_t>((prow + 3) / 4, 4096u)), dim3(256), 0, ctx->stream, patch_out, clip->w.cls, clip->w.pos, clip->w.pre_w,
                           clip->w.pre_b, (float *)nullptr, rows, T, d, Xn, AB, Xlo, rows_pad, lo8, (const uint32_t *)l0_list, (const uint32_t *)l0_cnt);
    } else
    hipLaunchKernelGGL(k_embed_ln, dim3((rows + 3) / 4), dim3(256), 0, ctx->stream, patch_out, clip->w.cls, clip->w.pos,
                       clip->w.pre_w, clip->w.pre_b, xf32 ? X : (float *)nullptr, rows, T, d, Xn, AB, Xlo, rows_pad, lo8);
    EpiAux ln = out_tm, st = a_tm;
    ln.a_rs = a_tm.a_rs;
    ln.a_ks = a_tm.a_ks;
    ln.ab = AB;
    st.hm_rows = rows_pad;
    st.xb = Xn;
    st.part = part;
    st.xlo = Xlo;
    const float inv_d = 1.0f / (float)d;
    uint32_t f8_first = D.num_layers, f8_end = D.num_layers;
    uint8_t *A8 = nullptr, *SA8 = nullptr, *AOS8 = nullptr, *H8 = nullptr, *SH8 = nullptr;
    uint32_t q8_grid = 0;
    if (ctx->vit_fp8 && split8 && d % 256 == 0 && mlp % 256 == 0 && mlp >= 2 * d) {
        f8_first = l0 ? 1u : 0u;
        f8_end = cls_last ? D.num_layers - 1 : D.num_layers;
        if (f8_first < f8_end) {
            if ((rc = ensure_f8_weights(ctx, (d2r_clip *)clip))) return rc;
            const size_t rp = rows_pad;
            AOS8 = (uint8_t *)AO + rp * d;
            H8 = (uint8_t *)H;
            SH8 = H8 + rp * mlp;
            A8 = SH8 + rp * (mlp / 64);
            SA8 = A8 + rp * d;
            q8_grid = (uint32_t)ctx->n_cu * 8u;
        }
    }
// ... 7 lines not shown
                return rc;
            const uint32_t n_pad = round_up(n, BM);
            uint16_t *Xq = H, *Qc = H + (size_t)n_pad * d;
            float2 *ABq = part;
            hipLaunchKernelGGL(k_gather_cls_operand, dim3((n * (d / 8) + 255) / 256), dim3(256), 0, ctx->stream, Xn, AB, rows_pad, T, d, n, Xq, ABq);
            EpiAux lq{};
            lq.cs = L.cs_qkv;
            lq.ab = ABq;
            if ((rc = launch_gemm<EPI_LN_BIAS_BF16>(ctx, Xq, L.wf_qkv, L.bf_qkv, Qc, n, d, d, lq))) return rc;
            if ((rc = last_block_cls(ctx, D, L, n, T, rows_pad, QKV, Qc, X, xf32 ? nullptr : Xn, Xlo, patch_out, AO, Xn, H, lo8))) return rc;
            break;
        }
        if (f8_first <= l && l < f8_end) {
            const d2r_clip::F8Layer &F = clip->f8[l];
            hipLaunchKernelGGL(k_ln_q8, dim3(q8_grid), dim3(256), 0, ctx->stream, Xn, AB, L.ln1_w, L.ln1_b, rows_pad, d, A8, SA8);
            if ((rc = launch_gemm_f8<EPI_F8_BIAS_BF16>(ctx, A8, SA8, F.w_qkv, F.s_qkv, L.b_qkv, QKV, rows, 3 * d, d, out_tm))) return rc;
            launch_attention_vision(ctx, QKV, AO, T, d, rows_pad, D.num_heads, n, AOS8);
            if ((rc = launch_gemm_f8<EPI_F8_RESID_STATS_SPLIT8>(ctx, (const uint8_t *)AO, AOS8, F.w_o, F.s_o, L.b_o, Xn, rows, d, d, st))) return rc;
            hipLaunchKernelGGL(k_rowstats, dim3((rows_pad + 255) / 256), dim3(256), 0, ctx->stream, part, np, rows_pad, inv_d, AB);
            hipLaunchKernelGGL(k_ln_q8, dim3(q8_grid), dim3(256), 0, ctx->stream, Xn, AB, L.ln2_w, L.ln2_b, rows_pad, d, A8, SA8);
            EpiAux hq = out_tm;
            hq.q8 = H8;
            hq.q8_scale = SH8;
            if ((rc = launch_gemm_f8<EPI_F8_BIAS_GELU_Q8>(ctx, A8, SA8, F.w_fc1, F.s_fc1, L.b_fc1, nullptr, rows, mlp, d, hq))) return rc;
            if ((rc = launch_gemm_f8<EPI_F8_RESID_STATS_SPLIT8>(ctx, H8, SH8, F.w_fc2, F.s_fc2, L.b_fc2, Xn, rows, d, mlp, st))) return rc;
            if (l + 1 < D.num_layers)
                hipLaunchKernelGGL(k_rowstats, dim3((rows_pad + 255) / 256), dim3(256), 0, ctx->stream, part, np, rows_pad, inv_d, AB);
            continue;
        }
        if (l0 && l == 0) {
            const uint32_t planes = 3 * d / 64;
            const size_t pieces = (size_t)planes * rows * 8;
            hipLaunchKernelGGL(k_bcast_qkv, dim3((uint32_t)((pieces + 255) / 256)), dim3(256), 0, ctx->stream, reuse->bg_qkv, reuse->bg_rows, QKV, rows, rows_pad, T, planes);
            float2 *AB2 = (float2 *)((uint8_t *)ctx->l0_misc.p + 256 + (size_t)prow * 4);
            hipLaunchKernelGGL(k_gather_operand_rows, dim3(2048), dim3(256), 0, ctx->stream, Xn, AB, rows_pad, T, (const uint32_t *)l0_list, (const uint32_t *)l0_cnt,
                               AO, AB2, cap_pad, d);
            EpiAux l2 = ln;
            l2.a_ks = 64 * cap_pad;
            l2.hm_rows = cap_pad;
            l2.ab = AB2;
            l2.m_dev = l0_cnt;
            if ((rc = launch_gemm_cfg<EPI_LN_BIAS_BF16, 4, 2, 2, 3>(ctx, AO, L.wf_qkv, L.bf_qkv, ctx->l0_q2.p, prow, 3 * d, d, l2))) return rc;
            hipLaunchKernelGGL(k_scatter_qkv, dim3(8192), dim3(256), 0, ctx->stream, (const uint16_t *)ctx->l0_q2.p, cap_pad, (const uint32_t *)l0_list,
                               (const uint32_t *)l0_cnt, QKV, rows_pad, T, planes);
        } else {
            const size_t tq = ctx->timing_begin(D2R_T_VIT_QKV);
            if ((rc = launch_gemm<EPI_LN_BIAS_BF16>(ctx, Xn, L.wf_qkv, L.bf_qkv, QKV, rows, 3 * d, d, ln))) return rc;
            ctx->timing_end(tq);
        }
        size_t tk = ctx->timing_begin(D2R_T_VIT_ATTN);
        launch_attention_vision(ctx, QKV, AO, T, d, rows_pad, D.num_heads, n);
        ctx->timing_end(tk);
        tk = ctx->timing_begin(D2R_T_VIT_OUT);
        if (xf32) rc = launch_gemm<EPI_RESID_STATS_F32X>(ctx, AO, L.w_o, L.b_o, X, rows, d, d, st);
        else if (split8) rc = launch_gemm<EPI_RESID_STATS_SPLIT8>(ctx, AO, L.w_o, L.b_o, Xn, rows, d, d, st);
        else if (split) rc = launch_gemm<EPI_RESID_STATS_SPLIT>(ctx, AO, L.w_o, L.b_o, Xn, rows, d, d, st);
        else rc = launch_gemm<EPI_RESID_STATS_BF16>(ctx, AO, L.w_o, L.b_o, Xn, rows, d, d, st);
        if (rc) return rc;
        ctx->timing_end(tk);
        hipLaunchKernelGGL(k_rowstats, dim3((rows_pad + 255) / 256), dim3(256), 0, ctx->stream, part, np, rows_pad, inv_d, AB);
        ln.cs = L.cs_fc1;
        tk = ctx->timing_begin(D2R_T_VIT_FC1);
        if ((rc = launch_gemm<EPI_LN_BIAS_GELU_BF16>(ctx, Xn, L.wf_fc1, L.bf_fc1, H, rows, mlp, d, ln))) return rc;
        ctx->timing_end(tk);
        tk = ctx->timing_begin(D2R_T_VIT_FC2);
        if (xf32) rc = launch_gemm<EPI_RESID_STATS_F32X>(ctx, H, L.w_fc2, L.b_fc2, X, rows, d, mlp, st);
        else if (split8) rc = launch_gemm<EPI_RESID_STATS_SPLIT8>(ctx, H, L.w_fc2, L.b_fc2, Xn, rows, d, mlp, st);
        else if (split) rc = launch_gemm<EPI_RESID_STATS_SPLIT>(ctx, H, L.w_fc2, L.b_fc2, Xn, rows, d, mlp, st);
        else rc = launch_gemm<EPI_RESID_STATS_BF16>(ctx, H, L.w_fc2, L.b_fc2, Xn, rows, d, mlp, st);
        if (rc) return rc;
        ctx->timing_end(tk);
        if (l + 1 < D.num_layers)
            hipLaunchKernelGGL(k_rowstats, dim3((rows_pad + 255) / 256), dim3(256), 0, ctx->stream, part, np, rows_pad, inv_d, AB);
    }
    if (cls_last)
        hipLaunchKernelGGL(k_head, dim3((n + HEAD_NI - 1) / HEAD_NI), dim3(HEAD_THREADS), 0, ctx->stream, patch_out, (const uint16_t *)nullptr, (const uint16_t *)nullptr, rows_pad,
                           (const uint32_t *)nullptr, 1u, d, clip->w.post_w, clip->w.post_b, clip->w.proj, D.proj_dim, text_dev, C, logit_scale, logits_dev,
                           embeds_dev, n);
    else
    hipLaunchKernelGGL(k_head, dim3((n + HEAD_NI - 1) / HEAD_NI), dim3(HEAD_THREADS), 0, ctx->stream, X, xf32 ? (const uint16_t *)nullptr : (const uint16_t *)Xn,
                       (const uint16_t *)Xlo, rows_pad, (const uint32_t *)nullptr, T, d, clip->w.post_w, clip->w.post_b, clip->w.proj, D.proj_dim, text_dev, C,
                       logit_scale, logits_dev, embeds_dev, n, lo8);
    D2R_HIP(ctx, hipGetLastError());
    return D2R_OK;
}

int d2r_launch_patchify(d2r_ctx *ctx, const d2r_clip *clip, const float *pv_dev, uint32_t n, uint16_t *patches_dev)
{
    size_t total = (size_t)n * 3 * clip->desc.image_size * clip->desc.image_size;
    hipLaunchKernelGGL(k_patchify, dim3((uint32_t)((total + 255) / 256)), dim3(256), 0, ctx->stream, pv_dev, n,
                       clip->desc.image_size, clip->desc.patch_size, patches_dev, clip->Kp_pad);
    D2R_HIP(ctx, hipGetLastError());
    return D2R_OK;
}

uint32_t d2r_clip_tokens(const d2r_clip *clip) { return clip->T; }

uint32_t d2r_clip_max_images(const d2r_clip *clip)
{
    const uint64_t widest = std::max<uint64_t>(3ull * clip->desc.hidden_size, clip->desc.mlp_size);
    const uint64_t rows = (0xffffffffull / widest) / BM * BM;
    return (uint32_t)std::max<uint64_t>(1, rows / clip->T);
}

size_t d2r_clip_patch_bytes(const d2r_clip *clip, uint32_t n)
{
    return (size_t)round_up(n * (clip->T - 1), BM) * clip->Kp_pad * 2;
}


extern "C" int d2r_clip_create(d2r_ctx *ctx, const d2r_clip_desc *desc, const float *weights, size_t n_floats,
                               d2r_clip **out)
{
    if (!ctx || !desc || !weights || !out) return d2r_fail(ctx, D2R_ERR_INVALID, "null argument");
    const uint32_t d = desc->hidden_size, P = desc->patch_size, S = desc->image_size, mlp = desc->mlp_size;
    if (d % 128 || mlp % 128 || d > 1024 || desc->proj_dim > 1024 || d / desc->num_heads != 64 || S % P)
        return d2r_fail(ctx, D2R_ERR_UNSUPPORTED, "unsupported CLIP geometry (need head_dim 64, d,mlp % 128 == 0, d <= 1024)");
    D2R_HIP(ctx, hipSetDevice(ctx->device));
    d2r_clip *c = new d2r_clip();
    c->ctx = ctx;
    c->desc = *desc;
    c->T = (S / P) * (S / P) + 1;
    c->Kp = 3 * P * P;
    c->Kp_pad = round_up(c->Kp, BK);
    const uint32_t T = c->T, Dp = desc->proj_dim;
    size_t expect = (size_t)d * c->Kp + d + (size_t)T * d + 2 * d +
                    (size_t)desc->num_layers * (4 * (size_t)d + 4 * ((size_t)d * d + d) + (size_t)mlp * d + mlp + (size_t)d * mlp + d) +
                    2 * d + (size_t)Dp * d;
    if (n_floats != expect) {
        delete c;
        return d2r_fail(ctx, D2R_ERR_INVALID, "weight blob size does not match the descriptor");
    }
    float *blob = nullptr;
    if (hipMalloc(&blob, n_floats * 4) != hipSuccess) {
        delete c;
        return d2r_fail(ctx, D2R_ERR_MEMORY, "hipMalloc failed for CLIP weights");
    }
    c->allocs.push_back(blob);
    if (hipMemcpy(blob, weights, n_floats * 4, hipMemcpyHostToDevice) != hipSuccess) {
        d2r_clip_destroy(c);
        return d2r_fail(ctx, D2R_ERR_DEVICE, "weight upload failed");
    }
    size_t off = 0;
    auto f32 = [&](size_t n) { const float *p = blob + off; off += n; return p; };
    bool ok = true;
    auto bf16 = [&](const float *src, uint32_t rows, uint32_t K, uint32_t K_pad) -> const uint16_t * {
        uint16_t *p = nullptr;
        if (hipMalloc(&p, (size_t)rows * K_pad * 2) != hipSuccess) { ok = false; return nullptr; }
        c->allocs.push_back(p);
        size_t tot = (size_t)rows * K_pad;
        hipLaunchKernelGGL(k_convert_bf16, dim3((uint32_t)((tot + 255) / 256)), dim3(256), 0, ctx->stream, src, p, rows, K, K_pad);
        return p;
    };
    c->w.w_patch = bf16(f32((size_t)d * c->Kp), d, c->Kp, c->Kp_pad);
    c->w.cls = f32(d);
    c->w.pos = f32((size_t)T * d);
    c->w.pre_w = f32(d);
    c->w.pre_b = f32(d);
    c->layers.resize(desc->num_layers);
    for (uint32_t l = 0; l < desc->num_layers && ok; l++) {
        ClipWeights::Layer &L = c->layers[l];
        L.ln1_w = f32(d);
        L.ln1_b = f32(d);
        uint16_t *wqkv = nullptr;
        float *bqkv = nullptr;
        if (hipMalloc(&wqkv, (size_t)3 * d * d * 2) != hipSuccess || hipMalloc(&bqkv, (size_t)3 * d * 4) != hipSuccess) { ok = false; break; }
// ... 284 lines not shown
```

dream2real_amd/csrc/d2r_internal.h:

```cpp
#pragma once
#include <hip/hip_runtime.h>
#include <stdint.h>

#include <functional>
#include <memory>
#include <mutex>
#include <string>
#include <utility>
#include <vector>

#include "../../include/d2r.h"
#include "d2r_shared.h"
#include "tsdf_sample.h"

class D2rJobPool;
struct D2rPngBase;

#define D2R_MAX_LEVELS 16
#define D2R_MAX_DEVICES 64
#define D2R_GRID 128
#define D2R_DT 0.0016914558f
#define D2R_INV_DT (1.0f / D2R_DT)
#define D2R_CONE 0.00390625f
#define D2R_T_LINEAR (D2R_DT * 256.0f)
#define D2R_N_WFRAG 24

struct LevelMeta {
    float scale;
    uint32_t res;
    uint32_t size;
    uint32_t offset;
    uint32_t hashed;
};

struct SlotMeta {
    float scale[2];
    uint32_t res[2];
    uint32_t size[2];
    uint32_t hashed[2];
    uint32_t mask8;
    uint32_t off;
    uint32_t bnx[2], bnxy[2];
    int32_t bbase[2];
};

struct NerfParams {
    const uint32_t *grid;
    uint32_t grid_bytes;
    uint32_t n_levels;
    int32_t n_dense;
    SlotMeta slot[D2R_MAX_LEVELS / 2];
    uint32_t refill_min;
    uint32_t compact;
    uint32_t sort_log2;
    uint32_t n_brick_slots;
    uint32_t brick_words;
    const uint32_t *brick_tab;
    uint32_t n_gbrick_slots;
    uint32_t gbrick_bytes;
    const uint32_t *gbrick_tab;
    const uint64_t *bricks;
    uint32_t aabb_scale;
    uint32_t n_casc;
    float side, inv_side;
    const uint4 *wfrag;
    const uint4 *wfrag16;
    float bbox_lo[3], bbox_hi[3];
    float raabb_lo[3], raabb_hi[3], rn_lo[3], rn_hi[3];
};

struct ViewParams {
    uint32_t W, H;
    float focal[2], center[2];
    float scale, inv_scale;
    float offset[3];
    float background[4];
    float min_transmittance, near_distance;
    uint32_t lens_mode;
    float lens[4];
    const float2 *lens_tab;
};

struct ClipParams;

struct D2rThumbPlan {
    bool valid = false;
    uint32_t n = 0, w = 0, h = 0, dilate_k = 0;
    size_t o_rgb = 0, o_mask = 0, o_oob = 0;
    uint64_t total = 0;
    std::vector<uint32_t> recs;
};

struct ClipL0Reuse {
    const void *rects;
    uint32_t w, h;
    const uint16_t *bg_hi;
    const uint8_t *bg_lo;
    const float2 *bg_ab;
    const uint16_t *bg_qkv;
    uint32_t bg_rows;
    uint32_t *touched_out;
};

struct d2r_ctx {
    int device = 0;
    hipStream_t own_stream = nullptr;
    hipStream_t stream = nullptr;
    std::string err;
    using Buf = D2rBuf;
    Buf queue2, sort_counts;
    Buf cams, queue, counters, frames, rgba, depth, poses, clipws[8], text, logits, pix;
    void *text_host[2] = {nullptr, nullptr};
    size_t text_host_cap[2] = {0, 0};
    hipEvent_t text_ev[2] = {nullptr, nullptr};
    uint32_t text_turn = 0;
    Buf bg_rgba, bg_depth, bg_u8;
    Buf pcd_mats, pcd_bg_keys, pcd_bg_frame, pcd_cols;
    Buf tv_mats, tv_bg_frame, tv_bg_depth, tv_depth;
    D2rStageTimer tv_timer, tv_pass_timer;
    D2rStageTimer tv_dl_timer;
    double tv_cast_ms = 0.0, tv_dl_ms = 0.0;
    bool tv_pass_pending = false, tv_dl_pending = false;
    Buf ct_in, ct_ws;
    D2rStageTimer ct_timer, ct_it_timer;
    double ct_ms[3] = {0.0, 0.0, 0.0};
    bool ct_timed = false;
    Buf lt_in, lt_ws;
    D2rStageTimer lt_timer;
    Buf gp_in, gp_ws;
    D2rStageTimer gp_timer, gp_timer2;
    Buf mv_in, mv_recs, mv_queue, mv_shade, mv_keys, mv_out;
    Buf mask_in, mask_out, mask_ws;
    Buf thumb_in, thumb_ws, thumb_out;
    D2rThumbPlan thumb_plan;
    D2rStageTimer thumb_timer[2];
    Buf prop_in, prop_ws, prop_out;
    D2rStageTimer prop_timer;
    D2rStageTimer mask_timer;
    D2rStageTimer pcdb_timer;
    Buf lens_tab;
    float lens_key[10] = {};
    bool lens_key_valid = false;
    Buf rect_ws;
    Buf rects;
    Buf bg_patches;
    const void *bg_patches_for = nullptr;
    Buf bg_l0, l0_a1, l0_q2, l0_misc;
    const void *bg_l0_for = nullptr;
    ClipL0Reuse bg_l0_desc{};
    int64_t vit_fp8 = 0;
    int64_t l0_reuse = 1;
    int64_t prep_reuse = 1;
    uint32_t bg_w = 0, bg_h = 0;
    d2r_render_stats stats{};
    int n_cu = 256, n_xcd = 8;
    void *comm = nullptr;
    int comm_rank = 0, comm_world = 1;
    hipStream_t render_stream = nullptr, copy_stream = nullptr;
    hipEvent_t ev_fork = nullptr, ev_prep[2] = {nullptr, nullptr}, ev_clip[2] = {nullptr, nullptr},
               ev_march[2] = {nullptr, nullptr}, ev_copy[2] = {nullptr, nullptr};
    Buf patches2, frames2;
    void *frame_host[2] = {nullptr, nullptr};
    size_t frame_host_cap[2] = {0, 0};
    D2rJobPool *pool = nullptr;
    std::shared_ptr<const D2rPngBase> png_base;
    int64_t overlap = 0;
    int64_t debug_fail_chunk = -1;
    uint32_t last_chunks = 0;
    int64_t chunk = 4096;
    uint32_t last_pass = 0;
    int64_t march_blocks = 0;
    int64_t ray_sort = 1;
    int64_t ray_sort_log2 = 4;
    int64_t march_threads = 0;
    int64_t march_threads_auto_mib = 64;
    int64_t last_march_threads = 0, last_march_gbrick_bytes = 0;
    int64_t last_march_nb = 0, last_march_ngb = 0;
    int64_t refill_min = 64;
    int64_t march_compact = 1;
    int64_t ln_fold = 4;
    int64_t gemm_nsplit = 0;
    int64_t attn_rem = 1;
    int64_t cls_last = 1;
    int64_t mlp_f16 = 1;
    int64_t render_arith = 0;
    int64_t use_bricks = 1;
    int64_t raygen_rect = 1;
    int64_t gbrick_slots = 8;
    int64_t brick_slots_total = 7;
    int64_t lds_slots_max = 5;
    int64_t gbrick_max_mib = 512;
    int64_t timing = 0;
    std::vector<hipEvent_t> ev_pool;
    size_t ev_used = 0;
    std::vector<std::pair<int, std::pair<size_t, size_t>>> ev_pairs;
    size_t timing_begin(int kind);
    void timing_end(size_t pair);
};
enum { D2R_T_MARCH = 0, D2R_T_RAYGEN = 1, D2R_T_CLIP = 2, D2R_T_PREP = 3, D2R_T_SORT = 4,
       D2R_T_VIT_QKV = 5, D2R_T_VIT_ATTN = 6, D2R_T_VIT_OUT = 7, D2R_T_VIT_FC1 = 8, D2R_T_VIT_FC2 = 9, D2R_T_KINDS = 10 };

struct d2r_nerf {
    d2r_ctx *ctx;
    int device = 0;
    NerfParams P{};
    D2rDev<uint32_t> d_grid, d_brick_tab, d_gbrick_tab;
    D2rDev<uint64_t> d_bricks;
    D2rDev<uint4> d_wfrag;
};

struct d2r_pcd {
    int device = 0;
    uint32_t n = 0;
    D2rDev<float4> xyz;
    D2rDev<uint32_t> rgb;
};

struct PerDeviceOnce {
    std::once_flag flag[D2R_MAX_DEVICES];
    template <class F>
    void run(int device, F &&fn) { std::call_once(flag[device % D2R_MAX_DEVICES], fn); }
};

bool d2r_tsdf_has_colour(const d2r_tsdf *v);
int d2r_tsdf_device(const d2r_tsdf *v);
float d2r_tsdf_voxel(const d2r_tsdf *v);
int d2r_tsdf_dev(d2r_ctx *ctx, d2r_tsdf *v, D2rTsdfDev *out);

int d2r_pcd_check_view(d2r_ctx *ctx, const d2r_pcd_view *view);

int d2r_phys_orientations(d2r_ctx *, const d2r_phys_params *, uint32_t N, uint64_t *oris_out);
std::vector<uint8_t> d2r_phys_orientation_mask(const d2r_phys_params *, const float *pose_batch, const uint8_t *valid_io, uint32_t oris);

struct d2r_clip;
uint32_t d2r_pass_size(const d2r_ctx *, const d2r_clip *clip, size_t px);
uint32_t d2r_frame_pass_size(uint32_t per, size_t px);
int d2r_upload_text(d2r_ctx *, const d2r_clip *, const float *text, uint32_t C);
int d2r_score_frames_chunked(d2r_ctx *, const d2r_clip *, uint32_t n, uint32_t w, uint32_t h, int rot90, uint32_t C, float logit_scale,
                             const std::function<int(uint32_t c0, uint32_t nc)> &fill, float *logits_out, float *embeds_out ,
                             uint8_t *frames_out );

int d2r_launch_cameras_direct(d2r_ctx *, const ViewParams &, const float *cams_nerf_dev, uint32_t n,
                              float *cams_out);
int d2r_launch_cameras_virtual(d2r_ctx *, const ViewParams &, const float *obj_now16,
                               const float *cam16, const float *obj_poses_dev, uint32_t n,
                               float *cams_out);
int d2r_launch_render(d2r_ctx *, const d2r_nerf *, const ViewParams &, const float *cams_dev,
                      uint32_t n, bool composite, float *rgba_dev, float *depth_dev,
                      uint8_t *frames_dev, void *rects_dev = nullptr);
int d2r_launch_bg_quantize(d2r_ctx *, uint32_t w, uint32_t h);
ViewParams d2r_view_params(const d2r_view *v);
int d2r_reserve_render(d2r_ctx *, size_t rays);
int d2r_lens_table(d2r_ctx *, ViewParams &V);
```

dream2real_amd/csrc/nerf.hip:

```cpp
#include <algorithm>
#include <cstring>

#include "d2r_internal.h"
#include <type_traits>

typedef __bf16 bf16x8 __attribute__((ext_vector_type(8)));
typedef float f32x16 __attribute__((ext_vector_type(16)));

typedef _Float16 f16x8 __attribute__((ext_vector_type(8)));
union Frag {
    bf16x8 v;
    f16x8 h;
    uint4 u;
};

template <bool F16>
__device__ __forceinline__ uint32_t pack2(float a, float b)
{
    if constexpr (F16) {
        typedef _Float16 f16x2 __attribute__((ext_vector_type(2)));
        union { f16x2 v; uint32_t u; } r;
        r.v[0] = (_Float16)a;
        r.v[1] = (_Float16)b;
        return r.u;
// ... 368 lines not shown
            }
            n = (int)floorf(dist / lattice_dt<CONE>(t + fmaxf(dist, 0.f)));
        } else {
            n = (int)floorf(dist * D2R_INV_DT);
        }
        k += (uint32_t)max(n, 1);
    }
    return false;
}

#define D2R_SORT_SHIFT 20
__device__ __forceinline__ uint32_t sort_tag(const NerfParams &P, float x, float y, float z)
{
    if (P.sort_log2 == 0) return 0u;
    const uint32_t n1 = 1u << P.sort_log2;
    uint32_t c[3];
    const float p[3] = {x, y, z};
#pragma unroll
    for (int a = 0; a < 3; a++) {
        const float u = (p[a] - P.bbox_lo[a]) / (P.bbox_hi[a] - P.bbox_lo[a]) * (float)n1;
        c[a] = min((uint32_t)fmaxf(u, 0.f), n1 - 1u);
    }
    uint32_t bin = 0;
#pragma unroll
    for (int b = 0; b < 4; b++) bin |= (((c[0] >> b) & 1u) << (3 * b)) | (((c[1] >> b) & 1u) << (3 * b + 1)) | (((c[2] >> b) & 1u) << (3 * b + 2));
    return bin << D2R_SORT_SHIFT;
}

__device__ __forceinline__ void empty_pixel(const ViewParams &V, float *rgba)
{
    rgba[0] = V.background[3] * V.background[0];
    rgba[1] = V.background[3] * V.background[1];
    rgba[2] = V.background[3] * V.background[2];
    rgba[3] = V.background[3];
}

template <bool CONE>
__global__ __launch_bounds__(256) void k_raygen(NerfParams P, ViewParams V, const float *__restrict__ cams,
                                                uint2 *__restrict__ queue, uint32_t *__restrict__ qcount,
                                                float *__restrict__ rgba_out, float *__restrict__ depth_out)
{
    if (CONE) cone_tab_to_lds();
    const uint32_t tiles_x = (V.W + 15) / 16;
    const uint32_t lane = threadIdx.x & 63, wave = threadIdx.x >> 6;
    const uint32_t px = (blockIdx.x % tiles_x) * 16 + (wave & 1) * 8 + (lane & 7);
    const uint32_t py = (blockIdx.x / tiles_x) * 16 + (wave >> 1) * 8 + (lane >> 3);
    const uint32_t cam_i = blockIdx.y;
    const bool inside = px < V.W && py < V.H;
    bool alive = false;
    uint32_t k = 0;
    if (inside) {
        float cam[12];
#pragma unroll
        for (int j = 0; j < 12; j++) cam[j] = cams[(size_t)cam_i * 12 + j];
        Ray r;
        if (make_ray<CONE>(P, V, cam, px, py, r, k)) {
            float x, y, z;
            alive = next_sample<CONE>(P, r, k, x, y, z);
            if (alive) k |= sort_tag(P, x, y, z);
        }
    }
    const uint32_t ray_id = cam_i * (V.W * V.H) + py * V.W + px;
    unsigned long long m = __ballot(alive);
    if (m) {
        uint32_t cnt = (uint32_t)__popcll(m), base = 0;
        if (lane == (uint32_t)__ffsll((long long)m) - 1) base = atomicAdd(qcount, cnt);
        base = __shfl(base, __ffsll((long long)m) - 1);
        if (alive) {
            uint32_t off = (uint32_t)__popcll(m & ((1ull << lane) - 1ull));
            queue[base + off] = make_uint2(ray_id, k);
        }
    }
    if (inside && !alive && rgba_out) {
        float e[4];
        empty_pixel(V, e);
        *(float4 *)(rgba_out + (size_t)ray_id * 4) = make_float4(e[0], e[1], e[2], e[3]);
        depth_out[ray_id] = 0.f;
    }
}

template <bool CONE>
__global__ __launch_bounds__(256) void k_raygen_rect(NerfParams P, ViewParams V, const float *__restrict__ cams,
                                                     uint2 *__restrict__ queue, uint32_t *__restrict__ qcount,
                                                     int4 *__restrict__ rects)
{
    if (CONE) cone_tab_to_lds();
    const uint32_t cam_i = blockIdx.x;
    const uint32_t lane = threadIdx.x & 63, wave = threadIdx.x >> 6;
    float cam[12];
#pragma unroll
    for (int j = 0; j < 12; j++) cam[j] = cams[(size_t)cam_i * 12 + j];
    int x0 = 0, y0 = 0, x1 = (int)V.W - 1, y1 = (int)V.H - 1;
    {
        bool ok = true;
#pragma unroll
        for (int a = 0; a < 3; a++)
#pragma unroll
            for (int b = a; b < 3; b++) {
                const float dot = cam[a] * cam[b] + cam[4 + a] * cam[4 + b] + cam[8 + a] * cam[8 + b];
                ok = ok && fabsf(dot - (a == b ? 1.0f : 0.0f)) < 1e-3f;
            }
        float u0 = INFINITY, u1 = -INFINITY, v0 = INFINITY, v1 = -INFINITY;
#pragma unroll
        for (int c = 0; c < 8; c++) {
            const float wx = (c & 1) ? P.bbox_hi[0] : P.bbox_lo[0], wy = (c & 2) ? P.bbox_hi[1] : P.bbox_lo[1];
            const float wz = (c & 4) ? P.bbox_hi[2] : P.bbox_lo[2];
            const float qx = (CONE ? fmaf(wx - 0.5f, P.side, 0.5f) : wx) - cam[3];
            const float qy = (CONE ? fmaf(wy - 0.5f, P.side, 0.5f) : wy) - cam[7];
            const float qz = (CONE ? fmaf(wz - 0.5f, P.side, 0.5f) : wz) - cam[11];
            const float cx = cam[0] * qx + cam[4] * qy + cam[8] * qz;
            const float cy = cam[1] * qx + cam[5] * qy + cam[9] * qz;
            const float cz = cam[2] * qx + cam[6] * qy + cam[10] * qz;
            ok = ok && cz > 1e-3f;
            const float un = cx / cz, vn = cy / cz;
            u0 = fminf(u0, un); u1 = fmaxf(u1, un);
            v0 = fminf(v0, vn); v1 = fmaxf(v1, vn);
        }
        ok = ok && u1 - u0 < 1e6f && v1 - v0 < 1e6f;
        float margin = 2.f;
        if (ok && V.lens_mode == D2R_LENS_OPENCV) {
            const uint32_t e = lane >> 4;
            const float s_ = (float)(lane & 15u) * (1.0f / 15.0f);
            const float bu = e == 0 ? fmaf(s_, u1 - u0, u0) : e == 1 ? u1 : e == 2 ? fmaf(s_, u1 - u0, u0) : u0;
            const float bv = e == 0 ? v0 : e == 1 ? fmaf(s_, v1 - v0, v0) : e == 2 ? v1 : fmaf(s_, v1 - v0, v0);
            float du, dv;
            lens_delta(V.lens, bu, bv, du, dv);
            float lu0 = bu + du, lu1 = lu0, lv0 = bv + dv, lv1 = lv0;
            const float k1 = V.lens[0], k2 = V.lens[1], p1 = V.lens[2], p2 = V.lens[3];
            const float r2 = bu * bu + bv * bv;
            const float rad = k1 * r2 + k2 * r2 * r2, drad = 2.f * k1 + 4.f * k2 * r2;
            const float jxx = 1.f + rad + bu * bu * drad + 2.f * p1 * bv + 6.f * p2 * bu;
            const float jxy = bu * bv * drad + 2.f * p1 * bu + 2.f * p2 * bv;
            const float jyy = 1.f + rad + bv * bv * drad + 2.f * p2 * bu + 6.f * p1 * bv;
            float detmin = jxx * jyy - jxy * jxy;
#pragma unroll
            for (int m = 32; m >= 1; m >>= 1) {
                lu0 = fminf(lu0, __shfl_xor(lu0, m)); lu1 = fmaxf(lu1, __shfl_xor(lu1, m));
                lv0 = fminf(lv0, __shfl_xor(lv0, m)); lv1 = fmaxf(lv1, __shfl_xor(lv1, m));
                detmin = fminf(detmin, __shfl_xor(detmin, m));
            }
            const float R = sqrtf(fmaxf(u0 * u0, u1 * u1) + fmaxf(v0 * v0, v1 * v1));
            const float d2max = 6.f * fabsf(k1) * R + 20.f * fabsf(k2) * R * R * R + 6.f * (fabsf(p1) + fabsf(p2));
            const float h = fmaxf(u1 - u0, v1 - v0) * (1.0f / 15.0f);
            margin += h * h * 0.125f * d2max * fmaxf(V.focal[0], V.focal[1]);
            ok = ok && detmin > 0.1f && margin < 1e6f;
            u0 = lu0; u1 = lu1; v0 = lv0; v1 = lv1;
        }
        if (ok) {
            const float pxmin = fmaf(u0, V.focal[0], V.center[0] * (float)V.W) - 0.5f, pxmax = fmaf(u1, V.focal[0], V.center[0] * (float)V.W) - 0.5f;
            const float pymin = fmaf(v0, V.focal[1], V.center[1] * (float)V.H) - 0.5f, pymax = fmaf(v1, V.focal[1], V.center[1] * (float)V.H) - 0.5f;
            const int mg = (int)ceilf(margin);
            x0 = max(x0, (int)floorf(fmaxf(pxmin, -4.f)) - mg);
            y0 = max(y0, (int)floorf(fmaxf(pymin, -4.f)) - mg);
            x1 = min(x1, (int)ceilf(fminf(pxmax, (float)V.W + 4.f)) + mg);
            y1 = min(y1, (int)ceilf(fminf(pymax, (float)V.H + 4.f)) + mg);
        }
    }
    if (x0 > x1 || y0 > y1) {
        if (rects && blockIdx.y == 0 && threadIdx.x == 0) rects[cam_i] = make_int4(1, 1, 0, 0);
        return;
    }
    const int tx0 = x0 >> 4, ty0 = y0 >> 4, ntx = (x1 >> 4) - tx0 + 1, nty = (y1 >> 4) - ty0 + 1;
    if (rects && blockIdx.y == 0 && threadIdx.x == 0)
        rects[cam_i] = make_int4(tx0 * 16, ty0 * 16, min((int)V.W, (tx0 + ntx) * 16) - 1, min((int)V.H, (ty0 + nty) * 16) - 1);
    constexpr uint32_t CAP = 2048;
    __shared__ uint2 pending[CAP];
    __shared__ uint32_t n_pending, flush_base;
    if (threadIdx.x == 0) n_pending = 0;
    __syncthreads();
    auto flush = [&]() {
        __syncthreads();
        const uint32_t np_ = n_pending;
        if (threadIdx.x == 0 && np_) flush_base = atomicAdd(qcount, np_);
        __syncthreads();
        for (uint32_t i = threadIdx.x; i < np_; i += 256) queue[flush_base + i] = pending[i];
        __syncthreads();
        if (threadIdx.x == 0) n_pending = 0;
        __syncthreads();
    };
    uint32_t since_flush = 0;
    for (int t = (int)blockIdx.y; t < ntx * nty; t += (int)gridDim.y) {
        if (since_flush + 256 > CAP) {
            flush();
            since_flush = 0;
        }
        since_flush += 256;
        const uint32_t px = (uint32_t)(tx0 + t % ntx) * 16 + (wave & 1) * 8 + (lane & 7);
        const uint32_t py = (uint32_t)(ty0 + t / ntx) * 16 + (wave >> 1) * 8 + (lane >> 3);
        bool alive = false;
        uint32_t k = 0;
        if (px < V.W && py < V.H) {
            Ray r;
            if (make_ray<CONE>(P, V, cam, px, py, r, k)) {
                float x, y, z;
                alive = next_sample<CONE>(P, r, k, x, y, z);
                if (alive) k |= sort_tag(P, x, y, z);
            }
        }
        const uint32_t ray_id = cam_i * (V.W * V.H) + py * V.W + px;
        unsigned long long m = __ballot(alive);
        if (m) {
            uint32_t cnt = (uint32_t)__popcll(m), base = 0;
            if (lane == (uint32_t)__ffsll((long long)m) - 1) base = atomicAdd(&n_pending, cnt);
            base = __shfl(base, __ffsll((long long)m) - 1);
            if (alive) {
                uint32_t off = (uint32_t)__popcll(m & ((1ull << lane) - 1ull));
                pending[base + off] = make_uint2(ray_id, k);
            }
        }
    }
    flush();
}

#define D2R_SORT_CHUNK 16384u
#define D2R_SORT_BINS 4096u
__global__ __launch_bounds__(256) void k_sort_count(const uint2 *__restrict__ queue, const uint32_t *__restrict__ qcount, uint32_t *__restrict__ counts)
{
    __shared__ uint32_t hist[D2R_SORT_BINS];
    const uint32_t n = *qcount, nchunks = (n + D2R_SORT_CHUNK - 1) / D2R_SORT_CHUNK;
    for (uint32_t c = blockIdx.x; c < nchunks; c += gridDim.x) {
        for (uint32_t i = threadIdx.x; i < D2R_SORT_BINS; i += 256) hist[i] = 0;
        __syncthreads();
        for (uint32_t i = c * D2R_SORT_CHUNK + threadIdx.x; i < min(n, (c + 1) * D2R_SORT_CHUNK); i += 256) atomicAdd(&hist[queue[i].y >> D2R_SORT_SHIFT], 1u);
        __syncthreads();
        for (uint32_t i = threadIdx.x; i < D2R_SORT_BINS; i += 256) counts[(size_t)i * nchunks + c] = hist[i];
        __syncthreads();
    }
}
__global__ __launch_bounds__(256) void k_sort_scan_rows(const uint32_t *__restrict__ qcount, uint32_t *__restrict__ counts, uint32_t *__restrict__ bin_total)
{
    const uint32_t n = *qcount, nchunks = (n + D2R_SORT_CHUNK - 1) / D2R_SORT_CHUNK;
    uint32_t *row = counts + (size_t)blockIdx.x * nchunks;
    const uint32_t total = d2r_block_scan_row(row, row, nchunks);
    if (threadIdx.x == 0) bin_total[blockIdx.x] = total;
}
__global__ __launch_bounds__(256) void k_sort_scan_bins(const uint32_t *__restrict__ bin_total, uint32_t *__restrict__ bin_base)
{
    d2r_block_scan_row(bin_total, bin_base, D2R_SORT_BINS);
}
__global__ __launch_bounds__(256) void k_sort_scatter(const uint2 *__restrict__ queue, const uint32_t *__restrict__ qcount, const uint32_t *__restrict__ counts,
// ... 669 lines not shown
    out[3 * (size_t)i + 0] = (uint8_t)q0;
    out[3 * (size_t)i + 1] = (uint8_t)q1;
    out[3 * (size_t)i + 2] = (uint8_t)q2;
}


ViewParams d2r_view_params(const d2r_view *v)
{
    ViewParams V;
    V.W = v->width;
    V.H = v->height;
    V.focal[0] = v->focal[0];
    V.focal[1] = v->focal[1];
    V.center[0] = v->center[0];
    V.center[1] = v->center[1];
    V.scale = v->scale;
    V.inv_scale = 1.0f / v->scale;
    for (int i = 0; i < 3; i++) V.offset[i] = v->offset[i];
    for (int i = 0; i < 4; i++) V.background[i] = v->background[i];
    V.min_transmittance = v->min_transmittance;
    V.near_distance = v->near_distance;
    V.lens_mode = v->lens_mode;
    for (int i = 0; i < 4; i++) V.lens[i] = v->lens_mode ? v->lens_params[i] : 0.f;
    V.lens_tab = nullptr;
    return V;
}

int d2r_launch_cameras_direct(d2r_ctx *ctx, const ViewParams &V, const float *cams_nerf_dev, uint32_t n,
                              float *cams_out)
{
    hipLaunchKernelGGL(k_cameras_direct, dim3((n + 63) / 64), dim3(64), 0, ctx->stream, V, cams_nerf_dev, n,
                       cams_out);
    D2R_HIP(ctx, hipGetLastError());
    return D2R_OK;
}

int d2r_launch_cameras_virtual(d2r_ctx *ctx, const ViewParams &V, const float *obj_now16, const float *cam16,
                               const float *obj_poses_dev, uint32_t n, float *cams_out)
{
    Mat16 a, b;
    for (int i = 0; i < 16; i++) {
        a.v[i] = obj_now16[i];
        b.v[i] = cam16[i];
    }
    hipLaunchKernelGGL(k_cameras_virtual, dim3((n + 63) / 64), dim3(64), 0, ctx->stream, V, a, b,
                       obj_poses_dev, n, cams_out);
    D2R_HIP(ctx, hipGetLastError());
    return D2R_OK;
}

int d2r_lens_table(d2r_ctx *ctx, ViewParams &V)
{
    V.lens_tab = nullptr;
    if (V.lens_mode != D2R_LENS_OPENCV) return D2R_OK;
    const float key[10] = {(float)V.W, (float)V.H, V.focal[0], V.focal[1], V.center[0], V.center[1], V.lens[0], V.lens[1], V.lens[2], V.lens[3]};
    const size_t px = (size_t)V.W * V.H;
    if (!ctx->lens_tab.p || !ctx->lens_key_valid || memcmp(key, ctx->lens_key, sizeof key) != 0) {
        ctx->lens_key_valid = false;
        int rc = d2r_reserve(ctx, ctx->lens_tab, px * sizeof(float2));
        if (rc) return rc;
        hipLaunchKernelGGL(k_lens_table, dim3((uint32_t)((px + 255) / 256)), dim3(256), 0, ctx->stream, V, (float2 *)ctx->lens_tab.p);
        D2R_HIP(ctx, hipGetLastError());
        D2R_HIP(ctx, hipStreamSynchronize(ctx->stream));
        memcpy(ctx->lens_key, key, sizeof key);
        ctx->lens_key_valid = true;
    }
    V.lens_tab = (const float2 *)ctx->lens_tab.p;
    return D2R_OK;
}

int d2r_reserve_render(d2r_ctx *ctx, size_t rays)
{
    int rc;
    if ((rc = d2r_reserve(ctx, ctx->queue, rays * sizeof(uint2)))) return rc;
    if (ctx->ray_sort) {
        const size_t max_chunks = (rays + D2R_SORT_CHUNK - 1) / D2R_SORT_CHUNK;
        if ((rc = d2r_reserve(ctx, ctx->queue2, rays * sizeof(uint2)))) return rc;
        if ((rc = d2r_reserve(ctx, ctx->sort_counts, (max_chunks + 2) * D2R_SORT_BINS * 4))) return rc;
    }
    return D2R_OK;
}

int d2r_launch_render(d2r_ctx *ctx, const d2r_nerf *m, const ViewParams &V, const float *cams_dev, uint32_t n,
                      bool composite, float *rgba_dev, float *depth_dev, uint8_t *frames_dev, void *rects_dev)
{
    const size_t rays = (size_t)n * V.W * V.H;
    if (rays >= (1ull << 32)) return d2r_fail(ctx, D2R_ERR_INVALID, "too many rays in one pass");
    if (V.lens_mode == D2R_LENS_OPENCV && !V.lens_tab)
        return d2r_fail(ctx, D2R_ERR_INVALID, "d2r_launch_render: a view with a lens arrived without its table (d2r_lens_table)");
    int rc;
    if ((rc = d2r_reserve_render(ctx, rays))) return rc;
    if ((rc = d2r_reserve(ctx, ctx->counters, 64))) return rc;
    uint32_t *cnt = (uint32_t *)ctx->counters.p;
    D2R_HIP(ctx, hipMemsetAsync(cnt, 0, 32, ctx->stream));
    if (composite) {
        if (ctx->bg_w != V.W || ctx->bg_h != V.H || !ctx->bg_u8.p)
            return d2r_fail(ctx, D2R_ERR_INVALID, "d2r_set_background must be called for this view first");
        const uint32_t n_bytes = V.W * V.H * 3;
        if (n_bytes % 16 == 0) {
            const uint32_t n_vec = n_bytes / 16;
            hipLaunchKernelGGL(k_frames_init, dim3((n_vec + 255) / 256, n < 64 ? n : 64), dim3(256), 0, ctx->stream,
                               (const uint4 *)ctx->bg_u8.p, (uint4 *)frames_dev, n_vec, n);
        } else {
            hipLaunchKernelGGL(k_frames_init_bytes, dim3((n_bytes + 255) / 256, n < 64 ? n : 64), dim3(256), 0,
                               ctx->stream, (const uint8_t *)ctx->bg_u8.p, frames_dev, n_bytes, n);
        }
    }
    const uint32_t tiles = ((V.W + 15) / 16) * ((V.H + 15) / 16);
    const uint32_t sort_log2 = ctx->ray_sort ? (uint32_t)ctx->ray_sort_log2 : 0u;
    NerfParams PR = m->P;
    PR.sort_log2 = sort_log2;
    size_t tr = ctx->timing_begin(D2R_T_RAYGEN);
    const bool cone = m->P.aabb_scale >= 2;
    if (composite && ctx->raygen_rect) {
        if (cone) hipLaunchKernelGGL(k_raygen_rect<true>, dim3(n, 4), dim3(256), 0, ctx->stream, PR, V, cams_dev, (uint2 *)ctx->queue.p, cnt, (int4 *)rects_dev);
        else hipLaunchKernelGGL(k_raygen_rect<false>, dim3(n, 4), dim3(256), 0, ctx->stream, PR, V, cams_dev, (uint2 *)ctx->queue.p, cnt, (int4 *)rects_dev);
    } else {
        if (cone)
            hipLaunchKernelGGL(k_raygen<true>, dim3(tiles, n), dim3(256), 0, ctx->stream, PR, V, cams_dev, (uint2 *)ctx->queue.p,
                               cnt, composite ? nullptr : rgba_dev, composite ? nullptr : depth_dev);
        else
            hipLaunchKernelGGL(k_raygen<false>, dim3(tiles, n), dim3(256), 0, ctx->stream, PR, V, cams_dev, (uint2 *)ctx->queue.p,
                               cnt, composite ? nullptr : rgba_dev, composite ? nullptr : depth_dev);
    }
    ctx->timing_end(tr);
    const uint2 *q = (const uint2 *)ctx->queue.p;
    if (sort_log2) {
        size_t ts = ctx->timing_begin(D2R_T_SORT);
        const size_t max_chunks = (rays + D2R_SORT_CHUNK - 1) / D2R_SORT_CHUNK;
        uint32_t *counts = (uint32_t *)ctx->sort_counts.p, *bin_total = counts + max_chunks * D2R_SORT_BINS, *bin_base = bin_total + D2R_SORT_BINS;
        const int sb = (int)std::min<size_t>(max_chunks, 4096);
        hipLaunchKernelGGL(k_sort_count, dim3(sb), dim3(256), 0, ctx->stream, q, cnt, counts);
        hipLaunchKernelGGL(k_sort_scan_rows, dim3(D2R_SORT_BINS), dim3(256), 0, ctx->stream, cnt, counts, bin_total);
        hipLaunchKernelGGL(k_sort_scan_bins, dim3(1), dim3(256), 0, ctx->stream, bin_total, bin_base);
        hipLaunchKernelGGL(k_sort_scatter, dim3(sb), dim3(256), 0, ctx->stream, q, cnt, counts, bin_base, (uint2 *)ctx->queue2.p);
        q = (const uint2 *)ctx->queue2.p;
        ctx->timing_end(ts);
    }
    size_t tm = ctx->timing_begin(D2R_T_MARCH);
    int blocks = ctx->march_blocks > 0 ? (int)ctx->march_blocks : ctx->n_cu;
    const float *bgd = (const float *)ctx->bg_depth.p;
    unsigned long long *sc = (unsigned long long *)(cnt + 2);
    const bool bricks_ok = ctx->use_bricks && m->P.n_dense == 5;
    uint32_t nb = bricks_ok ? m->P.n_brick_slots : 0;
    uint32_t ngb = 0;
    if (bricks_ok) {
        const uint32_t cap_total = (uint32_t)std::max<int64_t>(ctx->brick_slots_total, nb);
        ngb = std::min<uint32_t>(std::min<uint32_t>((uint32_t)ctx->gbrick_slots, m->P.n_gbrick_slots), cap_total - nb);
        bool none = false;
        switch (nb) {
            case 5: ngb = std::min(ngb, 3u); break;
            case 4: ngb = ngb >= 3 ? 3 : ngb >= 2 ? 2 : 0; break;
            case 3: case 2: case 1:
                if (ngb >= 7 - nb) ngb = 7 - nb;
                else if (ngb >= 6 - nb) ngb = 6 - nb;
                else none = true;
                break;
            default: ngb = ngb >= 7 ? 7 : ngb >= 6 ? 6 : 0; break;
        }
        if (none) nb = ngb = 0;
    }
    const int arith = (int)ctx->render_arith;
    if (arith) nb = ngb = 0;
    NerfParams PP = m->P;
    PP.refill_min = (uint32_t)ctx->refill_min;
    PP.compact = (uint32_t)ctx->march_compact;
    const size_t lds = (size_t)D2R_N_WFRAG * 64 * 16 + (nb ? (size_t)m->P.brick_words * 4 : 0);
    uint32_t threads = D2R_MARCH_THREADS;
    if (ctx->march_threads > 0) threads = std::min<uint32_t>((uint32_t)ctx->march_threads, D2R_MARCH_THREADS);
    else if (!sort_log2 && ngb && m->P.gbrick_bytes > (size_t)ctx->march_threads_auto_mib << 20) threads = std::min<uint32_t>(512u, D2R_MARCH_THREADS);
#define D2R_MARCH_C(COMP, NB, NGB, ND, CONE)                            \
    do {                                                                \
        if (ctx->mlp_f16) D2R_MARCH_F(COMP, NB, NGB, ND, CONE, true, 0);   \
        else D2R_MARCH_F(COMP, NB, NGB, ND, CONE, false, 0);               \
    } while (0)
#define D2R_MARCH_F(COMP, NB, NGB, ND, CONE, F16, ARITH)                                                              \
    do {                                                                                                          \
        static PerDeviceOnce attr;                                                                                \
        attr.run(ctx->device, [] {                                                                                \
            (void)hipFuncSetAttribute((const void *)k_march<COMP, NB, NGB, ND, CONE, F16, ARITH>, hipFuncAttributeMaxDynamicSharedMemorySize, 160 * 1024 - (CONE ? 512 : 0));  \
        });                                                                                                       \
        hipLaunchKernelGGL((k_march<COMP, NB, NGB, ND, CONE, F16, ARITH>), dim3(blocks), dim3(threads), lds, ctx->stream, PP, V, cams_dev, q, \
                           cnt, cnt + 1, COMP ? nullptr : rgba_dev, COMP ? nullptr : depth_dev,                   \
                           COMP ? bgd : nullptr, COMP ? frames_dev : nullptr, sc);                                \
    } while (0)
#define D2R_MARCH_CASE(COMP, CONE, NB, NGB) else if (nb == NB && ngb == NGB) D2R_MARCH_C(COMP, NB, NGB, 5, CONE);
#define D2R_MARCH_PICK(COMP, CONE)                                      \
    do {                                                                \
        if (m->P.n_dense != 5) D2R_MARCH_C(COMP, 0, 0, -1, CONE);       \
        D2R_MARCH_CASE(COMP, CONE, 5, 3) D2R_MARCH_CASE(COMP, CONE, 5, 2) D2R_MARCH_CASE(COMP, CONE, 5, 1) D2R_MARCH_CASE(COMP, CONE, 5, 0) \
        D2R_MARCH_CASE(COMP, CONE, 4, 3) D2R_MARCH_CASE(COMP, CONE, 4, 2) D2R_MARCH_CASE(COMP, CONE, 4, 0)                                  \
        D2R_MARCH_CASE(COMP, CONE, 3, 4) D2R_MARCH_CASE(COMP, CONE, 3, 3)                                                                   \
        D2R_MARCH_CASE(COMP, CONE, 2, 5) D2R_MARCH_CASE(COMP, CONE, 2, 4)                                                                   \
        D2R_MARCH_CASE(COMP, CONE, 1, 6) D2R_MARCH_CASE(COMP, CONE, 1, 5)                                                                   \
        D2R_MARCH_CASE(COMP, CONE, 0, 7) D2R_MARCH_CASE(COMP, CONE, 0, 6)                                                                   \
        else D2R_MARCH_C(COMP, 0, 0, 5, CONE);                          \
    } while (0)
#define D2R_MARCH_HALF(COMP, CONE)                                      \
    do {                                                                \
// ... 56 lines not shown
```

dream2real_amd/engine.py:

```python
from __future__ import annotations

import ctypes as C
import dataclasses
import os

import numpy as np

from . import _lib
from .clip_model import pack_text_weights, pack_vision_weights
from .scene import LENS_OPENCV, LENS_PERSPECTIVE, NerfModel, View

Shade = "Shade"
Depth = "Depth"


class Context:

    def __init__(self, device: int = 0):
        self.lib = _lib.load()
        h = C.c_void_p()
        _lib.check(self.lib.d2r_ctx_create(device, C.byref(h)))
        self.h = h
        self.device = device

    def close(self):
        if getattr(self, "h", None):
            self.lib.d2r_ctx_destroy(self.h)
            self.h = None

    def __del__(self):
        try:
            self.close()
        except Exception:
            pass

    def check(self, rc):
        _lib.check(rc, self.h)

    def set_stream(self, hip_stream_ptr: int):
        self.check(self.lib.d2r_ctx_set_stream(self.h, hip_stream_ptr))

    def synchronize(self):
        self.check(self.lib.d2r_ctx_synchronize(self.h))

    def set_option(self, key: str, value: int):
        self.check(self.lib.d2r_ctx_set_option(self.h, key.encode(), value))

    def get_option(self, key: str) -> int:
        v = C.c_int64(0)
        self.check(self.lib.d2r_ctx_get_option(self.h, key.encode(), C.byref(v)))
        return int(v.value)

    def render_stats(self, collect_K: int | None = None) -> dict:
        if collect_K is not None:
            self.check(self.lib.d2r_collect_render_stats(self.h, collect_K))
        s = _lib.RenderStats()
        self.check(self.lib.d2r_get_render_stats(self.h, C.byref(s)))
        return {"rays_total": s.rays_total, "rays_alive": s.rays_alive, "samples": s.samples,
                "wave_iters": s.wave_iters, "l0_tokens": s.l0_tokens, "l0_touched": s.l0_touched}

    def timing(self) -> dict:
        t = _lib.Timing()
        self.check(self.lib.d2r_get_timing(self.h, C.byref(t)))
        return {k: getattr(t, k) for k, _ in t._fields_}

    def comm_unique_id(self) -> bytes:
        buf = C.create_string_buffer(_lib.COMM_ID_BYTES)
        _lib.check(self.lib.d2r_comm_get_unique_id(buf))
        return buf.raw

    def comm_init(self, id_blob: bytes | None, rank: int, world: int):
        if id_blob is not None:
            assert len(id_blob) == _lib.COMM_ID_BYTES
        self.check(self.lib.d2r_comm_init(self.h, id_blob, rank, world))

    def comm_destroy(self):
        self.check(self.lib.d2r_comm_destroy(self.h))

    def allgather_scores(self, local_dev_ptr: int, n_local: int, global_dev_ptr: int):
        self.check(self.lib.d2r_allgather_scores(self.h, local_dev_ptr, n_local, global_dev_ptr))

    def set_background(self, view: View, bg_rgba: np.ndarray, bg_depth: np.ndarray):
        a = np.ascontiguousarray(bg_rgba, np.float32)
        d = np.ascontiguousarray(bg_depth, np.float32)
        assert a.shape == (view.height, view.width, 4) and d.shape == (view.height, view.width)
        v = _lib.view_c(view)
        self.check(self.lib.d2r_set_background(self.h, C.byref(v), _lib.ptr(a), _lib.ptr(d)))

    def lens_undistort_view(self, view: View) -> np.ndarray:
        out = np.empty((view.height, view.width, 2), np.float32)
        v = _lib.view_c(view)
        self.check(self.lib.d2r_lens_undistort_view(self.h, C.byref(v), _lib.ptr(out)))
        return out

    def rectify_background_depth(self, depth, mask, width: int, height: int, return_mask: bool = False):
        d = np.asarray(depth)
        d = np.ascontiguousarray(d, np.float16 if d.dtype == np.float16 else np.float32)
        sh, sw = d.shape
        m = None
        if mask is not None:
            m = np.ascontiguousarray(np.asarray(mask).astype(np.uint8))
            assert m.shape == (sh, sw)
        out = np.empty((height, width), np.float32)
        mo = np.empty((height, width), np.uint8) if (return_mask and m is not None) else None
        self.check(self.lib.d2r_rectify_background_depth(
            self.h, _lib.ptr(d), 1 if d.dtype == np.float16 else 0, _lib.ptr(m), sw, sh, width, height, _lib.ptr(out), _lib.ptr(mo)))
        return (out, mo) if return_mask else out


class _Nerf:

    def __init__(self):
        self.render_min_transmittance = 0.01
        self.render_with_lens_distortion = False
        self.render_lens = dict(mode=LENS_PERSPECTIVE, params=(0.0, 0.0, 0.0, 0.0))


class Testbed:

    def __init__(self, ctx: Context, model: NerfModel, training_views=None, dataset_scale: float = 1.0,
                 dataset_offset=(0.0, 0.3, 0.5)):
        self.ctx = ctx
        self.model = model
        lv = model.levels
        self._keep = dict(
            scale=np.ascontiguousarray(lv.scale, np.float32), res=np.ascontiguousarray(lv.res, np.uint32),
            size=np.ascontiguousarray(lv.size, np.uint32), offset=np.ascontiguousarray(lv.offset, np.uint32),
            grid=np.ascontiguousarray(model.grid, np.float16), dw1=np.ascontiguousarray(model.dw1, np.float16),
            dw2=np.ascontiguousarray(model.dw2, np.float16), cw1=np.ascontiguousarray(model.cw1, np.float16),
            cw2=np.ascontiguousarray(model.cw2, np.float16), cw3=np.ascontiguousarray(model.cw3, np.float16),
            occ=np.ascontiguousarray(model.occ_bits, np.uint8))
        k = self._keep
        desc = _lib.NerfDesc(lv.n_levels, lv.n_features, _lib.ptr(k["scale"]), _lib.ptr(k["res"]),
                             _lib.ptr(k["size"]), _lib.ptr(k["offset"]), lv.n_entries, _lib.ptr(k["grid"]),
                             _lib.ptr(k["dw1"]), _lib.ptr(k["dw2"]), _lib.ptr(k["cw1"]), _lib.ptr(k["cw2"]),
                             _lib.ptr(k["cw3"]), _lib.ptr(k["occ"]), int(getattr(model, "aabb_scale", 1)),
                             (C.c_float * 6)(*([0.0] * 6 if getattr(model, "render_aabb", None) is None
                                               else [float(x) for x in model.render_aabb])))
        h = C.c_void_p()
        ctx.check(ctx.lib.d2r_nerf_create(ctx.h, C.byref(desc), C.byref(h)))
        self.h = h
        self._init_state(training_views, dataset_scale, dataset_offset)
# ... 220 lines not shown
```

include/d2r.h:

```cpp
#ifndef D2R_H
#define D2R_H

#include <stddef.h>
#include <stdint.h>

#ifdef __cplusplus
extern "C" {
#endif

#define D2R_API __attribute__((visibility("default")))
#define D2R_ABI_VERSION 10

typedef enum {
    D2R_OK = 0,
    D2R_ERR_INVALID = -1,
    D2R_ERR_DEVICE = -2,
    D2R_ERR_MEMORY = -3,
    D2R_ERR_UNSUPPORTED = -4
} d2r_status;

typedef struct d2r_ctx d2r_ctx;
typedef struct d2r_nerf d2r_nerf;
typedef struct d2r_clip d2r_clip;

// ... 91 lines not shown
    uint32_t hidden_size;
    uint32_t num_layers;
    uint32_t num_heads;
    uint32_t mlp_size;
    uint32_t proj_dim;
} d2r_clip_desc;

D2R_API int d2r_clip_create(d2r_ctx *ctx, const d2r_clip_desc *desc, const float *weights,
                            size_t n_floats, d2r_clip **out);
D2R_API void d2r_clip_destroy(d2r_clip *clip);

D2R_API int d2r_clip_score_frames(d2r_ctx *ctx, const d2r_clip *clip, const uint8_t *frames,
                                  uint32_t n, uint32_t w, uint32_t h, int rot90,
                                  const float *text_embeds, uint32_t C, float logit_scale,
                                  float *logits_out, float *embeds_out);

D2R_API int d2r_clip_preprocess(d2r_ctx *ctx, const d2r_clip *clip, const uint8_t *frames,
                                uint32_t n, uint32_t w, uint32_t h, int rot90,
                                float *pixel_values_out);

D2R_API int d2r_clip_embed_pixels(d2r_ctx *ctx, const d2r_clip *clip, const float *pixel_values,
                                  uint32_t n, float *embeds_out);

D2R_API int d2r_debug_gemm_fp8(d2r_ctx *ctx, const float *A, const float *W, const float *bias, uint32_t M, uint32_t N,
                               uint32_t K, int kind, float *out, uint8_t *a_q8, uint8_t *a_scales, float *w_scale_out,
                               uint8_t *out_q8, uint8_t *out_scales);


typedef struct {
    uint32_t vocab_size;
    uint32_t context_length;
    uint32_t hidden_size;
    uint32_t num_layers;
    uint32_t num_heads;
    uint32_t mlp_size;
    uint32_t proj_dim;
} d2r_text_desc;
typedef struct d2r_text d2r_text;

D2R_API int d2r_text_create(d2r_ctx *ctx, const d2r_text_desc *desc, const float *weights,
                            size_t n_floats, d2r_text **out);
D2R_API void d2r_text_destroy(d2r_text *text);
D2R_API int d2r_text_encode(d2r_ctx *ctx, const d2r_text *text, const int32_t *input_ids, uint32_t C,
                            uint32_t T, float *embeds_out);


D2R_API int d2r_render_score(d2r_ctx *ctx, const d2r_nerf *fg, const d2r_clip *clip,
                             const d2r_view *view, const float *obj_pose_now,
                             const float *cam_pose, const float *obj_poses_dev, uint32_t K,
                             const float *text_embeds, uint32_t C, float logit_scale,
                             float *logits_dev, uint8_t *frames_out);

typedef struct {
    const char *png_dir;
    uint32_t png_first_index;
    int32_t png_threads;
    int32_t png_level;
} d2r_frame_sink;

D2R_API int d2r_render_score_host(d2r_ctx *ctx, const d2r_nerf *fg, const d2r_clip *clip,
                                  const d2r_view *view, const float *obj_pose_now, const float *cam_pose,
                                  const float *obj_poses, uint32_t K, const float *text_embeds, uint32_t C,
                                  float logit_scale, float *logits_out, uint8_t *frames_out,
                                  const d2r_frame_sink *sink);


D2R_API int d2r_png_write(const uint8_t *rgb, uint32_t w, uint32_t h, const char *path, int level);
D2R_API int d2r_png_write_batch(const uint8_t *frames, uint32_t n, uint32_t w, uint32_t h, const char *dir,
                                uint32_t first_index, int threads, int level);
D2R_API int d2r_png_write_batch_bg(const uint8_t *frames, uint32_t n, uint32_t w, uint32_t h, const uint8_t *background, const char *dir,
                                   uint32_t first_index, int threads);
D2R_API int d2r_png_read_batch(const char *dir, const uint32_t *indices, uint32_t first_index, uint32_t n, uint32_t w,
                               uint32_t h, uint8_t *frames_out, int threads);
D2R_API int d2r_png_size(const char *path, uint32_t *w, uint32_t *h);
D2R_API int d2r_savetxt(const char *path, const double *data, uint64_t rows, uint64_t cols, int threads);

typedef struct {
    uint64_t rays_total;
    uint64_t rays_alive;
    uint64_t samples;
    uint64_t wave_iters;
    uint64_t l0_tokens;
    uint64_t l0_touched;
} d2r_render_stats;
D2R_API int d2r_get_render_stats(d2r_ctx *ctx, d2r_render_stats *out);
D2R_API int d2r_collect_render_stats(d2r_ctx *ctx, uint32_t K);

typedef struct {
    double march_ms;   uint64_t march_launches;
    double raygen_ms;  uint64_t raygen_launches;
    double prep_ms;    uint64_t prep_launches;
    double clip_ms;    uint64_t clip_launches;
    double sort_ms;    uint64_t sort_launches;
    double vit_qkv_ms;  uint64_t vit_qkv_launches;
    double vit_attn_ms; uint64_t vit_attn_launches;
    double vit_out_ms;  uint64_t vit_out_launches;
    double vit_fc1_ms;  uint64_t vit_fc1_launches;
    double vit_fc2_ms;  uint64_t vit_fc2_launches;
} d2r_timing;
D2R_API int d2r_get_timing(d2r_ctx *ctx, d2r_timing *out);

D2R_API int d2r_ctx_set_option(d2r_ctx *ctx, const char *key, int64_t value);
D2R_API int d2r_ctx_get_option(d2r_ctx *ctx, const char *key, int64_t *value);


#define D2R_COMM_ID_BYTES 128
D2R_API int d2r_comm_get_unique_id(void *id_out);
D2R_API int d2r_comm_init(d2r_ctx *ctx, const void *id_blob, int rank, int world);
D2R_API int d2r_comm_destroy(d2r_ctx *ctx);
D2R_API int d2r_allgather_scores(d2r_ctx *ctx, const float *local_dev, size_t n_local, float *global_dev);


typedef struct d2r_phys d2r_phys;
D2R_API int d2r_phys_create(d2r_ctx *ctx, const float *movable_verts, const uint32_t *movable_offsets, uint32_t n_movable,
                            const float *static_verts, const uint32_t *static_offsets, uint32_t n_static, d2r_phys **out);
D2R_API void d2r_phys_destroy(d2r_phys *phys);
typedef struct {
    uint32_t sample_res[6];
    float init_pose[16];
    float table_z;
    float unsup_thresh;
    float gravity[3];
    float perturb;
    int32_t stability_check;
    int32_t disallow_regrasp;
    float margin;
} d2r_phys_params;
D2R_API int d2r_phys_check(d2r_ctx *ctx, const d2r_phys *phys, const d2r_phys_params *params, const float *pose_batch,
                           uint32_t N, uint8_t *valid_io);

typedef struct d2r_pcd d2r_pcd;

D2R_API int d2r_pcd_create(d2r_ctx *ctx, const float *xyz, const uint8_t *rgb, uint32_t n, d2r_pcd **out);
D2R_API void d2r_pcd_destroy(d2r_pcd *pcd);

typedef struct {
    uint32_t width, height;
    float fx, fy, cx, cy;
    float point_size;
    float near;
} d2r_pcd_view;

D2R_API int d2r_pcd_render(d2r_ctx *ctx, const d2r_pcd *bg, const d2r_pcd *movable, const d2r_pcd_view *view,
                           const float *cam_pose, const float *obj_pose_now, const float *obj_poses, uint32_t K,
                           uint8_t *frames_out);

D2R_API int d2r_pcd_render_score_host(d2r_ctx *ctx, const d2r_pcd *bg, const d2r_pcd *movable, const d2r_clip *clip,
                                      const d2r_pcd_view *view, const float *cam_pose, const float *obj_pose_now,
                                      const float *obj_poses, uint32_t K, const float *text_embeds, uint32_t C,
                                      float logit_scale, float *logits_out, uint8_t *frames_out);

D2R_API int d2r_pcd_build(d2r_ctx *ctx, const uint8_t *rgb, const uint16_t *depth_u16, const uint8_t *labels, uint32_t n, uint32_t w,
                          uint32_t h, const double *cam_poses, const double *K, const double *bounds, double voxel,
                          const uint32_t *views, uint32_t n_views, const uint8_t *obj_ids, uint32_t n_objs, d2r_pcd **out);
D2R_API int d2r_pcd_size(const d2r_pcd *pcd, uint32_t *n);
D2R_API int d2r_pcd_read(d2r_ctx *ctx, const d2r_pcd *pcd, float *xyz, uint8_t *rgb);
D2R_API int d2r_pcd_build_get_timing(d2r_ctx *ctx, double *ms_out);

typedef struct d2r_tsdf d2r_tsdf;

D2R_API int d2r_tsdf_create(d2r_ctx *ctx, const float *bounds, float voxel, float trunc, d2r_tsdf **out);
D2R_API void d2r_tsdf_destroy(d2r_tsdf *vol);

D2R_API int d2r_tsdf_integrate(d2r_tsdf *vol, const uint16_t *depth_u16, const uint8_t *mask_u8, uint32_t w, uint32_t h,
                               const float *intrinsics, const float *cam_pose, uint32_t erode_k);

// ... 172 lines not shown
```

Baseline: 28400.

## Skip CLIP forward for candidates whose render leaves crop untouched; cull raygen to crop

Adds a device pass that lists candidates whose rendered rect touches any CLIP patch. Only those candidates plus the background image go through the CLIP forward, and each untouched candidate gets the background logits scattered back into its row. Raygen rects are also clamped to the pixel footprint the CLIP crop actually reads, so rays outside the crop are never marched. In exchange it adds a host sync on an event per chunk to read the touched count, plus extra small kernels; overlap between streams may suffer.

Result: no change. 28640, median of 6 (+0.8%).

```diff
diff --git a/dream2real_amd/_lib.py b/dream2real_amd/_lib.py
--- a/dream2real_amd/_lib.py
+++ b/dream2real_amd/_lib.py
@@ -175,7 +175,7 @@
 
 class RenderStats(C.Structure):
     _fields_ = [("rays_total", C.c_uint64), ("rays_alive", C.c_uint64), ("samples", C.c_uint64),
-                ("wave_iters", C.c_uint64), ("l0_tokens", C.c_uint64), ("l0_touched", C.c_uint64)]
+                ("wave_iters", C.c_uint64), ("l0_tokens", C.c_uint64), ("l0_touched", C.c_uint64), ("l0_skipped", C.c_uint64)]
 
 
 class Timing(C.Structure):
diff --git a/dream2real_amd/csrc/api.hip b/dream2real_amd/csrc/api.hip
--- a/dream2real_amd/csrc/api.hip
+++ b/dream2real_amd/csrc/api.hip
@@ -6,6 +6,7 @@
 
 #include "d2r_internal.h"
 #include "pngio.h"
+#include "skip_host.h"
 
 struct d2r_clip;
 int d2r_launch_preprocess(d2r_ctx *, d2r_clip *, const uint8_t *frames_dev, uint32_t n, uint32_t w, uint32_t h,
@@ -18,6 +19,10 @@
 int d2r_launch_patchify(d2r_ctx *, const d2r_clip *, const float *pv_dev, uint32_t n, uint16_t *patches_dev);
 size_t d2r_clip_patch_bytes(const d2r_clip *, uint32_t n);
 int d2r_launch_eval_points(d2r_ctx *, const d2r_nerf *, const float *xyz, const float *dirs, uint32_t n, float *out);
+int d2r_clip_image_list(d2r_ctx *, const d2r_clip *, const void *rects_dev, uint32_t n, uint32_t w, uint32_t h, uint32_t *cnt_dev, uint32_t *list_dev,
+                        uint32_t *slot_dev);
+int d2r_clip_scatter_rows(d2r_ctx *, const float *src_dev, const uint32_t *slot_dev, uint32_t bg_slot, uint32_t n, uint32_t cols, float *dst_dev);
+int d2r_clip_crop_footprint(d2r_ctx *, const d2r_clip *, uint32_t w, uint32_t h, int rot90, int out[4]);
 uint32_t d2r_clip_image_size(const d2r_clip *);
 uint32_t d2r_clip_proj_dim(const d2r_clip *);
 uint32_t d2r_clip_max_images(const d2r_clip *);
@@ -158,6 +163,8 @@
     {"cls_last", &d2r_ctx::cls_last, Option::FLAG},
     {"vit_fp8", &d2r_ctx::vit_fp8, Option::FLAG},
     {"l0_reuse", &d2r_ctx::l0_reuse, Option::FLAG},
+    {"skip_untouched", &d2r_ctx::skip_untouched, Option::FLAG},
+    {"crop_cull", &d2r_ctx::crop_cull, Option::FLAG},
     {"attn_rem", &d2r_ctx::attn_rem, Option::RANGE, 0, 4},
     {"overlap", &d2r_ctx::overlap, Option::FLAG},
     {"debug_fail_chunk", &d2r_ctx::debug_fail_chunk, Option::FREE},
@@ -284,7 +291,7 @@
     delete c->pool;
     d2r_ctx::Buf *bufs[] = {&c->cams, &c->queue, &c->queue2, &c->sort_counts, &c->counters, &c->frames, &c->rgba, &c->depth, &c->poses,
                             &c->text, &c->logits, &c->pix, &c->bg_rgba, &c->bg_depth, &c->bg_u8, &c->rects, &c->bg_patches, &c->rect_ws, &c->lens_tab,
-                            &c->patches2, &c->frames2, &c->bg_l0, &c->l0_a1, &c->l0_q2, &c->l0_misc,
+                            &c->patches2, &c->frames2, &c->bg_l0, &c->l0_a1, &c->l0_q2, &c->l0_misc, &c->skip_ws,
                             &c->pcd_mats, &c->pcd_bg_keys, &c->pcd_bg_frame, &c->pcd_cols,
                             &c->tv_mats, &c->tv_bg_frame, &c->tv_bg_depth, &c->tv_depth, &c->ct_in, &c->ct_ws, &c->lt_in, &c->lt_ws, &c->gp_in, &c->gp_ws,
                             &c->mv_in, &c->mv_recs, &c->mv_queue, &c->mv_shade, &c->mv_keys, &c->mv_out,
@@ -300,11 +307,12 @@
         if (c->text_host[k]) (void)hipHostFree(c->text_host[k]);
     }
     hipEvent_t evs[] = {c->ev_fork, c->ev_prep[0], c->ev_prep[1], c->ev_clip[0], c->ev_clip[1], c->ev_march[0], c->ev_march[1],
-                        c->ev_copy[0], c->ev_copy[1]};
+                        c->ev_copy[0], c->ev_copy[1], c->ev_skip[0], c->ev_skip[1]};
     for (hipEvent_t e : evs)
         if (e) (void)hipEventDestroy(e);
     for (int k = 0; k < 2; k++)
         if (c->frame_host[k]) (void)hipHostFree(c->frame_host[k]);
+    if (c->skip_host) (void)hipHostFree(c->skip_host);
     if (c->render_stream) (void)hipStreamDestroy(c->render_stream);
     if (c->copy_stream) (void)hipStreamDestroy(c->copy_stream);
     (void)hipStreamDestroy(c->own_stream);
@@ -847,7 +855,7 @@
     if (!ctx->render_stream) D2R_HIP(ctx, hipStreamCreateWithFlags(&ctx->render_stream, hipStreamNonBlocking));
     if (need_copy && !ctx->copy_stream) D2R_HIP(ctx, hipStreamCreateWithFlags(&ctx->copy_stream, hipStreamNonBlocking));
     hipEvent_t *all[] = {&ctx->ev_fork, &ctx->ev_prep[0], &ctx->ev_prep[1], &ctx->ev_clip[0], &ctx->ev_clip[1],
-                         &ctx->ev_march[0], &ctx->ev_march[1], &ctx->ev_copy[0], &ctx->ev_copy[1]};
+                         &ctx->ev_march[0], &ctx->ev_march[1], &ctx->ev_copy[0], &ctx->ev_copy[1], &ctx->ev_skip[0], &ctx->ev_skip[1]};
     for (hipEvent_t *e : all)
         if (!*e) D2R_HIP(ctx, hipEventCreateWithFlags(e, hipEventDisableTiming));
     return D2R_OK;
@@ -952,6 +960,18 @@
             l0.rects = ctx->rects.p;
         }
     }
+    const bool skip = l0.rects && ctx->skip_untouched;
+    const size_t skip_half = 256 + (size_t)cap * 8;
+    if (skip) {
+        if ((rc = d2r_reserve(ctx, ctx->skip_ws, 2 * skip_half + (size_t)cap * C * 4))) return rc;
+        if (!ctx->skip_host && hipHostMalloc((void **)&ctx->skip_host, 64, hipHostMallocDefault) != hipSuccess) {
+            ctx->skip_host = nullptr;
+            return d2r_fail(ctx, D2R_ERR_MEMORY, "hipHostMalloc failed for the skipped-candidate counts");
+        }
+    }
+    int cull[4];
+    const bool use_cull = ctx->crop_cull && ctx->raygen_rect && !to_host;
+    if (use_cull && (rc = d2r_clip_crop_footprint(ctx, clip, V.W, V.H, 1, cull))) return rc;
     ctx->stats = d2r_render_stats{};
     hipStream_t main = ctx->stream, rs = two ? ctx->render_stream : main, xs = ctx->copy_stream;
     if (rs != main) {
@@ -973,8 +993,14 @@
             if (two && ci >= 2) D2R_HIP(ctx, hipStreamWaitEvent(rs, ctx->ev_clip[pb], 0));
             if ((rc = d2r_launch_cameras_virtual(ctx, V, obj_pose_now, cam_pose, poses_dev + (size_t)c0 * 16, nc, (float *)ctx->cams.p)))
                 return rc;
-            if ((rc = d2r_launch_render(ctx, fg, V, (const float *)ctx->cams.p, nc, true, nullptr, nullptr, frames_dev, rects)))
+            if ((rc = d2r_launch_render(ctx, fg, V, (const float *)ctx->cams.p, nc, true, nullptr, nullptr, frames_dev, rects, use_cull ? cull : nullptr)))
                 return rc;
+            if (skip) {
+                uint32_t *sk = (uint32_t *)((uint8_t *)ctx->skip_ws.p + (size_t)pb * skip_half);
+                if ((rc = d2r_clip_image_list(ctx, clip, rects, nc, V.W, V.H, sk, sk + 64, sk + 64 + cap))) return rc;
+                D2R_HIP(ctx, hipMemcpyAsync(ctx->skip_host + pb, sk, 4, hipMemcpyDeviceToHost, rs));
+                D2R_HIP(ctx, hipEventRecord(ctx->ev_skip[pb], rs));
+            }
             D2R_HIP(ctx, hipMemcpyAsync((uint8_t *)ctx->counters.p + 64 + 32 * (size_t)ci, ctx->counters.p, 32,
                                         hipMemcpyDeviceToDevice, rs));
             if (ctx->debug_fail_chunk >= 0 && (int64_t)ci == ctx->debug_fail_chunk) {
@@ -1000,9 +1026,25 @@
             l0.rects = rects;
             l0.touched_out = (uint32_t *)((uint8_t *)ctx->counters.p + 64 + 32 * (size_t)ci) + 6;
         }
-        if ((rc = d2r_clip_forward(ctx, clip, patches, nc, (const float *)ctx->text.p, C, logit_scale,
-                                   logits_dev + (size_t)c0 * C, nullptr, l0.rects ? &l0 : nullptr)))
-            return rc;
+        D2rSkipPlan plan = d2r_skip_plan(nc, nc);
+        if (skip) {
+            D2R_HIP(ctx, hipEventSynchronize(ctx->ev_skip[pb]));
+            plan = d2r_skip_plan(nc, ctx->skip_host[pb]);
+            ctx->stats.l0_skipped += plan.skipped;
+        }
+        if (plan.compact) {
+            const uint32_t *sk = (const uint32_t *)((uint8_t *)ctx->skip_ws.p + (size_t)pb * skip_half);
+            float *compact = (float *)((uint8_t *)ctx->skip_ws.p + 2 * skip_half);
+            l0.img_list = sk + 64;
+            l0.n_listed = plan.n_listed;
+            if ((rc = d2r_clip_forward(ctx, clip, patches, plan.n_run, (const float *)ctx->text.p, C, logit_scale, compact, nullptr, &l0))) return rc;
+            if ((rc = d2r_clip_scatter_rows(ctx, compact, sk + 64 + cap, plan.n_listed, nc, C, logits_dev + (size_t)c0 * C))) return rc;
+        } else {
+            l0.img_list = nullptr;
+            if ((rc = d2r_clip_forward(ctx, clip, patches, nc, (const float *)ctx->text.p, C, logit_scale,
+                                       logits_dev + (size_t)c0 * C, nullptr, l0.rects ? &l0 : nullptr)))
+                return rc;
+        }
         ctx->timing_end(tc);
         if (two) D2R_HIP(ctx, hipEventRecord(ctx->ev_clip[pb], main));
         if (to_host) {
diff --git a/dream2real_amd/csrc/clip.hip b/dream2real_amd/csrc/clip.hip
--- a/dream2real_amd/csrc/clip.hip
+++ b/dream2real_amd/csrc/clip.hip
@@ -1,4 +1,5 @@
 #include "d2r_internal.h"
+#include "skip_host.h"
 
 #include <type_traits>
 
@@ -47,6 +48,7 @@
     uint32_t w, h;
     int rot90;
     ResampleTables R;
+    std::vector<int> bounds_h, bounds_v;
 };
 
 struct d2r_clip {
@@ -1470,35 +1472,103 @@
 }
 
 
+__device__ __forceinline__ void patch_rows(const ResampleTables &R, uint32_t P, uint32_t pr, int &ys, int &ye)
+{
+    if (R.need_v) {
+        ys = R.bounds_v[2 * (R.top + pr * P)];
+        const int last = R.top + pr * P + P - 1;
+        ye = R.bounds_v[2 * last] + R.bounds_v[2 * last + 1];
+    } else { ys = R.top + pr * P; ye = ys + P; }
+}
+__device__ __forceinline__ void patch_cols(const ResampleTables &R, uint32_t P, uint32_t pcol, int &xs, int &xe)
+{
+    if (R.need_h) {
+        xs = R.bounds_h[2 * (R.left + pcol * P)];
+        const int last = R.left + pcol * P + P - 1;
+        xe = R.bounds_h[2 * last] + R.bounds_h[2 * last + 1];
+    } else { xs = R.left + pcol * P; xe = xs + P; }
+}
+
 __global__ __launch_bounds__(256) void k_touch_list(const int4 *__restrict__ rects, uint32_t w, ResampleTables R, uint32_t S, uint32_t P,
-                                                    uint32_t *__restrict__ cnt, uint32_t *__restrict__ list)
+                                                    uint32_t *__restrict__ cnt, uint32_t *__restrict__ list,
+                                                    const uint32_t *__restrict__ img_list, uint32_t n_listed, uint32_t *__restrict__ src_list)
 {
     __shared__ uint32_t ids[1024], n_ids, base;
     const uint32_t img = blockIdx.x, g = S / P, g2 = g * g;
     if (threadIdx.x == 0) n_ids = 0;
     __syncthreads();
-    const int4 rc = rects[img];
+    if (img_list && img >= n_listed) return;
+    const uint32_t src = img_list ? img_list[img] : img;
+    const int4 rc = rects[src];
     const bool empty = rc.x > rc.z || rc.y > rc.w;
     const int rlo = (int)w - 1 - rc.z, rhi = (int)w - 1 - rc.x, clo = rc.y, chi = rc.w;
     for (uint32_t p = threadIdx.x; p < g2 && !empty; p += blockDim.x) {
         const uint32_t pr = p / g, pcol = p - pr * g;
         int ys, ye, xs, xe;
-        if (R.need_v) {
-            ys = R.bounds_v[2 * (R.top + pr * P)];
-            const int last = R.top + pr * P + P - 1;
-            ye = R.bounds_v[2 * last] + R.bounds_v[2 * last + 1];
-        } else { ys = R.top + pr * P; ye = ys + P; }
-        if (R.need_h) {
-            xs = R.bounds_h[2 * (R.left + pcol * P)];
-            const int last = R.left + pcol * P + P - 1;
-            xe = R.bounds_h[2 * last] + R.bounds_h[2 * last + 1];
-        } else { xs = R.left + pcol * P; xe = xs + P; }
-        if (!(rhi < ys || rlo >= ye || chi < xs || clo >= xe)) ids[atomicAdd(&n_ids, 1u)] = img * g2 + p;
+        patch_rows(R, P, pr, ys, ye);
+        patch_cols(R, P, pcol, xs, xe);
+        if (!(rhi < ys || rlo >= ye || chi < xs || clo >= xe)) ids[atomicAdd(&n_ids, 1u)] = p;
     }
     __syncthreads();
     if (threadIdx.x == 0) base = n_ids ? atomicAdd(cnt, n_ids) : 0u;
     __syncthreads();
-    for (uint32_t i = threadIdx.x; i < n_ids; i += blockDim.x) list[base + i] = ids[i];
+    for (uint32_t i = threadIdx.x; i < n_ids; i += blockDim.x) {
+        list[base + i] = img * g2 + ids[i];
+        if (src_list) src_list[base + i] = src * g2 + ids[i];
+    }
+}
+
+__global__ __launch_bounds__(1024) void k_image_list(const int4 *__restrict__ rects, uint32_t n, uint32_t w, ResampleTables R, uint32_t S, uint32_t P,
+                                                     uint32_t *__restrict__ cnt, uint32_t *__restrict__ list, uint32_t *__restrict__ slot)
+{
+    __shared__ uint32_t wave_tot[16];
+    const uint32_t g = S / P, lane = threadIdx.x & 63, wave = threadIdx.x >> 6;
+    uint32_t run = 0;
+    for (uint32_t b0 = 0; b0 < n; b0 += 1024) {
+        const uint32_t img = b0 + threadIdx.x;
+        bool touched = false;
+        if (img < n) {
+            const int4 rc = rects[img];
+            if (!(rc.x > rc.z || rc.y > rc.w)) {
+                const int rlo = (int)w - 1 - rc.z, rhi = (int)w - 1 - rc.x, clo = rc.y, chi = rc.w;
+                bool row = false, col = false;
+                for (uint32_t q = 0; q < g; q++) {
+                    int s, e;
+                    patch_rows(R, P, q, s, e);
+                    row = row || !(rhi < s || rlo >= e);
+                    patch_cols(R, P, q, s, e);
+                    col = col || !(chi < s || clo >= e);
+                }
+                touched = row && col;
+            }
+        }
+        const unsigned long long m = __ballot(touched);
+        if (lane == 0) wave_tot[wave] = (uint32_t)__popcll(m);
+        __syncthreads();
+        uint32_t before = 0, total = 0;
+        for (uint32_t k = 0; k < 16; k++) {
+            const uint32_t c = wave_tot[k];
+            before += k < wave ? c : 0u;
+            total += c;
+        }
+        if (img < n) {
+            const uint32_t pos = run + before + (uint32_t)__popcll(m & ((1ull << lane) - 1ull));
+            if (touched) list[pos] = img;
+            slot[img] = touched ? pos : 0xffffffffu;
+        }
+        run += total;
+        __syncthreads();
+    }
+    if (threadIdx.x == 0) *cnt = run;
+}
+
+__global__ __launch_bounds__(256) void k_scatter_rows(const float *__restrict__ src, const uint32_t *__restrict__ slot, uint32_t bg_slot, uint32_t n,
+                                                      uint32_t cols, float *__restrict__ dst)
+{
+    const size_t i = (size_t)blockIdx.x * blockDim.x + threadIdx.x;
+    if (i >= (size_t)n * cols) return;
+    const uint32_t r = (uint32_t)(i / cols), c = (uint32_t)(i - (size_t)r * cols), s = slot[r];
+    dst[i] = src[(size_t)(s == 0xffffffffu ? bg_slot : s) * cols + c];
 }
 
 __global__ __launch_bounds__(256) void k_gather_rows(const uint16_t *__restrict__ src, uint32_t row_elems, const uint32_t *__restrict__ list,
@@ -2430,7 +2500,7 @@
     R.kk_h = dev + o_kh;
     R.bounds_v = dev + o_bv;
     R.kk_v = dev + o_kv;
-    clip->prep.push_back(PrepCache{w, h, rot90, R});
+    clip->prep.push_back(PrepCache{w, h, rot90, R, bh, bv});
     *out = &clip->prep.back();
     return D2R_OK;
 }
@@ -2704,14 +2774,19 @@
     if (l0) {
         const PrepCache *pc = nullptr;
         if ((rc = prep_tables(ctx, (d2r_clip *)clip, reuse->w, reuse->h, 1, &pc))) return rc;
-        if ((rc = d2r_reserve(ctx, ctx->l0_misc, 256 + (size_t)prow * 4 + (size_t)cap_pad * 8))) return rc;
+        if ((rc = d2r_reserve(ctx, ctx->l0_misc, 256 + (size_t)prow * 8 + (size_t)cap_pad * 8))) return rc;
         if ((rc = d2r_reserve(ctx, ctx->l0_a1, (size_t)cap_pad * clip->Kp_pad * 2))) return rc;
         if ((rc = d2r_reserve(ctx, ctx->l0_q2, (size_t)cap_pad * 3 * d * 2))) return rc;
         l0_cnt = (uint32_t *)ctx->l0_misc.p;
         l0_list = l0_cnt + 64;
         D2R_HIP(ctx, hipMemsetAsync(l0_cnt, 0, 4, ctx->stream));
-        hipLaunchKernelGGL(k_touch_list, dim3(n), dim3(256), 0, ctx->stream, (const int4 *)reuse->rects, reuse->w, pc->R, D.image_size, D.patch_size, l0_cnt, l0_list);
-        hipLaunchKernelGGL(k_gather_rows, dim3(2048), dim3(256), 0, ctx->stream, patches_dev, clip->Kp_pad, l0_list, l0_cnt, (uint16_t *)ctx->l0_a1.p);
+        uint32_t *src_list = reuse->img_list ? (uint32_t *)((uint8_t *)ctx->l0_misc.p + 256 + (size_t)prow * 4 + (size_t)cap_pad * 8) : nullptr;
+        if (reuse->img_list && reuse->n_listed + 1 != n)
+            return d2r_fail(ctx, D2R_ERR_INVALID, "d2r_clip_forward: a compacted launch is its listed candidates and the background image");
+        hipLaunchKernelGGL(k_touch_list, dim3(n), dim3(256), 0, ctx->stream, (const int4 *)reuse->rects, reuse->w, pc->R, D.image_size, D.patch_size, l0_cnt, l0_list,
+                           reuse->img_list, reuse->n_listed, src_list);
+        hipLaunchKernelGGL(k_gather_rows, dim3(2048), dim3(256), 0, ctx->stream, patches_dev, clip->Kp_pad, src_list ? (const uint32_t *)src_list : (const uint32_t *)l0_list, l0_cnt,
+                           (uint16_t *)ctx->l0_a1.p);
         if (reuse->touched_out) D2R_HIP(ctx, hipMemcpyAsync(reuse->touched_out, l0_cnt, 4, hipMemcpyDeviceToDevice, ctx->stream));
         if (getenv("D2R_L0_DEBUG")) {
             uint32_t c = 0;
@@ -2885,6 +2960,37 @@
                        (const uint16_t *)Xlo, rows_pad, (const uint32_t *)nullptr, T, d, clip->w.post_w, clip->w.post_b, clip->w.proj, D.proj_dim, text_dev, C,
                        logit_scale, logits_dev, embeds_dev, n, lo8);
     D2R_HIP(ctx, hipGetLastError());
+    return D2R_OK;
+}
+
+int d2r_clip_image_list(d2r_ctx *ctx, const d2r_clip *clip, const void *rects_dev, uint32_t n, uint32_t w, uint32_t h, uint32_t *cnt_dev,
+                        uint32_t *list_dev, uint32_t *slot_dev)
+{
+    const PrepCache *pc = nullptr;
+    int rc = prep_tables(ctx, (d2r_clip *)clip, w, h, 1, &pc);
+    if (rc) return rc;
+    hipLaunchKernelGGL(k_image_list, dim3(1), dim3(1024), 0, ctx->stream, (const int4 *)rects_dev, n, w, pc->R, clip->desc.image_size, clip->desc.patch_size,
+                       cnt_dev, list_dev, slot_dev);
+    D2R_HIP(ctx, hipGetLastError());
+    return D2R_OK;
+}
+
+int d2r_clip_scatter_rows(d2r_ctx *ctx, const float *src_dev, const uint32_t *slot_dev, uint32_t bg_slot, uint32_t n, uint32_t cols, float *dst_dev)
+{
+    const size_t total = (size_t)n * cols;
+    if (!total) return D2R_OK;
+    hipLaunchKernelGGL(k_scatter_rows, dim3((uint32_t)((total + 255) / 256)), dim3(256), 0, ctx->stream, src_dev, slot_dev, bg_slot, n, cols, dst_dev);
+    D2R_HIP(ctx, hipGetLastError());
+    return D2R_OK;
+}
+
+int d2r_clip_crop_footprint(d2r_ctx *ctx, const d2r_clip *clip, uint32_t w, uint32_t h, int rot90, int out[4])
+{
+    const PrepCache *pc = nullptr;
+    int rc = prep_tables(ctx, (d2r_clip *)clip, w, h, rot90, &pc);
+    if (rc) return rc;
+    const ResampleTables &R = pc->R;
+    d2r_crop_footprint(pc->bounds_h.data(), R.need_h, R.left, pc->bounds_v.data(), R.need_v, R.top, (int)clip->desc.image_size, (int)w, (int)h, rot90, out);
     return D2R_OK;
 }
 
diff --git a/dream2real_amd/csrc/d2r_internal.h b/dream2real_amd/csrc/d2r_internal.h
--- a/dream2real_amd/csrc/d2r_internal.h
+++ b/dream2real_amd/csrc/d2r_internal.h
@@ -100,6 +100,8 @@
     const uint16_t *bg_qkv;
     uint32_t bg_rows;
     uint32_t *touched_out;
+    const uint32_t *img_list;
+    uint32_t n_listed;
 };
 
 struct d2r_ctx {
@@ -146,6 +148,11 @@
     Buf bg_patches;
     const void *bg_patches_for = nullptr;
     Buf bg_l0, l0_a1, l0_q2, l0_misc;
+    Buf skip_ws;
+    uint32_t *skip_host = nullptr;
+    hipEvent_t ev_skip[2] = {nullptr, nullptr};
+    int64_t skip_untouched = 1;
+    int64_t crop_cull = 1;
     const void *bg_l0_for = nullptr;
     ClipL0Reuse bg_l0_desc{};
     int64_t vit_fp8 = 0;
@@ -247,7 +254,8 @@
                                float *cams_out);
 int d2r_launch_render(d2r_ctx *, const d2r_nerf *, const ViewParams &, const float *cams_dev,
                       uint32_t n, bool composite, float *rgba_dev, float *depth_dev,
-                      uint8_t *frames_dev, void *rects_dev = nullptr);
+                      uint8_t *frames_dev, void *rects_dev = nullptr,
+                      const int *cull = nullptr);
 int d2r_launch_bg_quantize(d2r_ctx *, uint32_t w, uint32_t h);
 ViewParams d2r_view_params(const d2r_view *v);
 int d2r_reserve_render(d2r_ctx *, size_t rays);
diff --git a/dream2real_amd/csrc/nerf.hip b/dream2real_amd/csrc/nerf.hip
--- a/dream2real_amd/csrc/nerf.hip
+++ b/dream2real_amd/csrc/nerf.hip
@@ -474,7 +474,7 @@
 template <bool CONE>
 __global__ __launch_bounds__(256) void k_raygen_rect(NerfParams P, ViewParams V, const float *__restrict__ cams,
                                                      uint2 *__restrict__ queue, uint32_t *__restrict__ qcount,
-                                                     int4 *__restrict__ rects)
+                                                     int4 *__restrict__ rects, int4 cull)
 {
     if (CONE) cone_tab_to_lds();
     const uint32_t cam_i = blockIdx.x;
@@ -548,6 +548,8 @@
             y1 = min(y1, (int)ceilf(fminf(pymax, (float)V.H + 4.f)) + mg);
         }
     }
+    x0 = max(x0, cull.x); y0 = max(y0, cull.y);
+    x1 = min(x1, cull.z); y1 = min(y1, cull.w);
     if (x0 > x1 || y0 > y1) {
         if (rects && blockIdx.y == 0 && threadIdx.x == 0) rects[cam_i] = make_int4(1, 1, 0, 0);
         return;
@@ -1383,7 +1385,7 @@
 }
 
 int d2r_launch_render(d2r_ctx *ctx, const d2r_nerf *m, const ViewParams &V, const float *cams_dev, uint32_t n,
-                      bool composite, float *rgba_dev, float *depth_dev, uint8_t *frames_dev, void *rects_dev)
+                      bool composite, float *rgba_dev, float *depth_dev, uint8_t *frames_dev, void *rects_dev, const int *cull)
 {
     const size_t rays = (size_t)n * V.W * V.H;
     if (rays >= (1ull << 32)) return d2r_fail(ctx, D2R_ERR_INVALID, "too many rays in one pass");
@@ -1414,8 +1416,10 @@
     size_t tr = ctx->timing_begin(D2R_T_RAYGEN);
     const bool cone = m->P.aabb_scale >= 2;
     if (composite && ctx->raygen_rect) {
-        if (cone) hipLaunchKernelGGL(k_raygen_rect<true>, dim3(n, 4), dim3(256), 0, ctx->stream, PR, V, cams_dev, (uint2 *)ctx->queue.p, cnt, (int4 *)rects_dev);
-        else hipLaunchKernelGGL(k_raygen_rect<false>, dim3(n, 4), dim3(256), 0, ctx->stream, PR, V, cams_dev, (uint2 *)ctx->queue.p, cnt, (int4 *)rects_dev);
+        const int4 cl = cull ? make_int4(std::max(cull[0], 0), std::max(cull[1], 0), std::min(cull[2], (int)V.W - 1), std::min(cull[3], (int)V.H - 1))
+                             : make_int4(0, 0, (int)V.W - 1, (int)V.H - 1);
+        if (cone) hipLaunchKernelGGL(k_raygen_rect<true>, dim3(n, 4), dim3(256), 0, ctx->stream, PR, V, cams_dev, (uint2 *)ctx->queue.p, cnt, (int4 *)rects_dev, cl);
+        else hipLaunchKernelGGL(k_raygen_rect<false>, dim3(n, 4), dim3(256), 0, ctx->stream, PR, V, cams_dev, (uint2 *)ctx->queue.p, cnt, (int4 *)rects_dev, cl);
     } else {
         if (cone)
             hipLaunchKernelGGL(k_raygen<true>, dim3(tiles, n), dim3(256), 0, ctx->stream, PR, V, cams_dev, (uint2 *)ctx->queue.p,
diff --git a/dream2real_amd/csrc/skip_host.h b/dream2real_amd/csrc/skip_host.h
--- /dev/null
+++ b/dream2real_amd/csrc/skip_host.h
@@ -0,0 +1,55 @@
+#pragma once
+#include <limits.h>
+#include <stdint.h>
+
+static inline void d2r_read_interval(const int *bounds, int need, int first, int count, int src_size, int *lo, int *hi)
+{
+    int l = INT_MAX, h = INT_MIN;
+    if (!need) {
+        l = first;
+        h = first + count;
+    } else {
+        for (int i = first; i < first + count; i++) {
+            const int s = bounds[2 * i], n = bounds[2 * i + 1];
+            if (n <= 0) continue;
+            if (s < l) l = s;
+            if (s + n > h) h = s + n;
+        }
+    }
+    if (l < 0) l = 0;
+    if (h > src_size) h = src_size;
+    *lo = l;
+    *hi = h;
+}
+
+static inline void d2r_crop_footprint(const int *bounds_h, int need_h, int left, const int *bounds_v, int need_v, int top, int S,
+                                      int w, int h, int rot90, int out[4])
+{
+    const int iw = rot90 ? h : w, ih = rot90 ? w : h;
+    int clo, chi, rlo, rhi;
+    d2r_read_interval(bounds_h, need_h, left, S, iw, &clo, &chi);
+    d2r_read_interval(bounds_v, need_v, top, S, ih, &rlo, &rhi);
+    if (rot90) {
+        out[0] = w - rhi;
+        out[1] = clo;
+        out[2] = w - 1 - rlo;
+        out[3] = chi - 1;
+    } else {
+        out[0] = clo;
+        out[1] = rlo;
+        out[2] = chi - 1;
+        out[3] = rhi - 1;
+    }
+}
+
+struct D2rSkipPlan {
+    uint32_t n_run;
+    uint32_t n_listed;
+    uint32_t skipped;
+    bool compact;
+};
+static inline D2rSkipPlan d2r_skip_plan(uint32_t nc, uint32_t m)
+{
+    if (m >= nc) return D2rSkipPlan{nc, nc, 0u, false};
+    return D2rSkipPlan{m + 1u, m, nc - m, true};
+}
diff --git a/dream2real_amd/engine.py b/dream2real_amd/engine.py
--- a/dream2real_amd/engine.py
+++ b/dream2real_amd/engine.py
@@ -57,7 +57,7 @@
         s = _lib.RenderStats()
         self.check(self.lib.d2r_get_render_stats(self.h, C.byref(s)))
         return {"rays_total": s.rays_total, "rays_alive": s.rays_alive, "samples": s.samples,
-                "wave_iters": s.wave_iters, "l0_tokens": s.l0_tokens, "l0_touched": s.l0_touched}
+                "wave_iters": s.wave_iters, "l0_tokens": s.l0_tokens, "l0_touched": s.l0_touched, "l0_skipped": s.l0_skipped}
 
     def timing(self) -> dict:
         t = _lib.Timing()
diff --git a/include/d2r.h b/include/d2r.h
--- a/include/d2r.h
+++ b/include/d2r.h
@@ -197,6 +197,7 @@
     uint64_t wave_iters;
     uint64_t l0_tokens;
     uint64_t l0_touched;
+    uint64_t l0_skipped;
 } d2r_render_stats;
 D2R_API int d2r_get_render_stats(d2r_ctx *ctx, d2r_render_stats *out);
 D2R_API int d2r_collect_render_stats(d2r_ctx *ctx, uint32_t K);
```
